# zhoubin-me/agent0

Measured on AMD Instinct MI355X. Metric: env-frames/sec (learner FPS: transitions collected and saved to replay per second with the learner running, pre-frameskip), higher is better.
Workload: dtype f32

## Files before the change

### agent0_amd/csrc/a0_internal.h

```cpp
#pragma once
#include "../../include/agent0_hip.h"
#include "a0_defs.h"

#include <exception>
#if defined(__HIPCC__)
#include <hip/hip_ext.h>
#endif
#include <stdexcept>
#include <string>

int a0_fail(int code, const char* msg);
int a0_fail_hip(int hip_error, const char* what);

struct a0_hip_error : std::runtime_error {
    int err;
    a0_hip_error(int e, const std::string& w) : std::runtime_error(w), err(e) {}
};

#define A0_STR2(x) #x
#define A0_STR(x) A0_STR2(x)
#define A0_HIP_THROW(expr)                                                                                  \
    do {                                                                                                    \
        hipError_t a0_e_ = (expr);                                                                          \
        if (a0_e_ != hipSuccess) throw a0_hip_error((int)a0_e_, std::string(__FILE__ ":" A0_STR(__LINE__) ": ") + hipGetErrorString(a0_e_)); \
    } while (0)

#define A0_TRY try {
#define A0_CATCH                                                   \
    }                                                              \
    catch (const a0_hip_error& e) { return a0_fail_hip(e.err, e.what()); } \
    catch (const std::exception& e) { return a0_fail(A0_EINVAL, e.what()); } \
    catch (...) { return a0_fail(A0_EINVAL, "unknown C++ exception"); }

void a0_trace_push_internal(const char* name);
void a0_trace_pop_internal();
struct a0_trace_scope {
    explicit a0_trace_scope(const char* name) { a0_trace_push_internal(name); }
    ~a0_trace_scope() { a0_trace_pop_internal(); }
    a0_trace_scope(const a0_trace_scope&) = delete;
    a0_trace_scope& operator=(const a0_trace_scope&) = delete;
};

#if defined(__HIPCC__)
bool a0_probe_start(int tag, hipStream_t st);
struct a0_tail_prep;
int a0_conv1_wgrad_fused_launch(const a0_frames_arg* f, int C, int H, int W, int B, const float* d1, float* slabs, const a0_tail_prep* prep, hipStream_t st);
void a0_probe_stop(hipStream_t st, double flops);
bool a0_probe_events(int tag, hipEvent_t* start, hipEvent_t* stop);
void a0_probe_commit(double flops);
int a0_x9_products_now();
#define A0_LAUNCH_PROBED(tag, flops, kern, grid, block, lds, st, ...)                                                              \
    do {                                                                                                                           \
        hipEvent_t a0_e0_ = nullptr, a0_e1_ = nullptr;                                                                             \
        if (a0_probe_events((tag), &a0_e0_, &a0_e1_)) {                                                                            \
            hipExtLaunchKernelGGL(kern, grid, block, (uint32_t)(lds), st, a0_e0_, a0_e1_, 0, __VA_ARGS__);                         \
            a0_probe_commit(flops);                                                                                                \
        } else                                                                                                                     \
            hipLaunchKernelGGL(kern, grid, block, lds, st, __VA_ARGS__);                                                           \
    } while (0)
struct a0_net_core;
int a0_conv23_wgrad_fused_launch(const a0_net_core& n, int B, const float* act1, const float* act2, const float* d2, const float* d3, float* slab2, float* slab3,
                                 hipStream_t st);
#endif
#define A0_TAG_ENCODER_FUSED 12
#define A0_TAG_ENCODER_DGRAD_FUSED 13
#define A0_TAG_ACTOR_STEP_ENC 14
```

### agent0_amd/csrc/conv23_wgrad.hip

```cpp
#include "a0_internal.h"
#include "net_impl.h"

#include <cstdlib>

typedef __bf16 a0q_bf16x8 __attribute__((ext_vector_type(8)));
typedef short a0q_s16x4 __attribute__((ext_vector_type(4)));
typedef uint32_t a0q_u32x2 __attribute__((ext_vector_type(2)));
typedef uint32_t a0q_u32x4 __attribute__((ext_vector_type(4)));
typedef float a0_acc16 __attribute__((ext_vector_type(16)));

constexpr int A0Q_THREADS = 512;
constexpr int A0Q_ROW = 64;

struct a0_c23w_args {
    const float *act1, *act2, *d2, *d3;
    float *slab2, *slab3;
    int B, G2, G3;
};

template <int LAYER> struct a0q_geom;
template <> struct a0q_geom<2> {
    static constexpr int NPOS = 81, STEPS = 5, DROWS = 96, APIX = 100, CIN = 32, K = 512;
    static constexpr int ACT_PLANE = APIX * A0Q_ROW, D_PLANE = 2 * DROWS * A0Q_ROW;
    static constexpr int ACT_F4 = 100 * 8, D_F4 = 81 * 16;
    A0_D static int base_row(int p) { return 10 * (p / 9) + (p % 9); }
};
template <> struct a0q_geom<3> {
    static constexpr int NPOS = 49, STEPS = 3, DROWS = 64, APIX = 81, CIN = 64, K = 576;
    static constexpr int ACT_PLANE = 2 * APIX * A0Q_ROW, D_PLANE = 2 * DROWS * A0Q_ROW;
    static constexpr int ACT_F4 = 81 * 16, D_F4 = 49 * 16;
    A0_D static int base_row(int p) { return 9 * (p / 7) + (p % 7); }
};
constexpr int A0Q_LDS_BYTES = 3 * (a0q_geom<2>::ACT_PLANE + a0q_geom<2>::D_PLANE);
static_assert(3 * (a0q_geom<3>::ACT_PLANE + a0q_geom<3>::D_PLANE) <= A0Q_LDS_BYTES && 2 * A0Q_LDS_BYTES <= 160 * 1024, "conv3 image fits; two workgroups per CU");

A0_D void a0q_split4(const a0_f4& v, a0q_u32x2& hi, a0q_u32x2& mid, a0q_u32x2& lo) {
    const float x[4] = {v.x, v.y, v.z, v.w};
    uint32_t h[4], m[4], l[4];
#pragma unroll
    for (int e = 0; e < 4; ++e) {
        h[e] = __float_as_uint(x[e]);
        const float r1 = x[e] - __uint_as_float(h[e] & 0xffff0000u);
        m[e] = __float_as_uint(r1);
        l[e] = __float_as_uint(r1 - __uint_as_float(m[e] & 0xffff0000u));
    }
    hi.x = __builtin_amdgcn_perm(h[1], h[0], 0x07060302u);  hi.y = __builtin_amdgcn_perm(h[3], h[2], 0x07060302u);
    mid.x = __builtin_amdgcn_perm(m[1], m[0], 0x07060302u); mid.y = __builtin_amdgcn_perm(m[3], m[2], 0x07060302u);
    lo.x = __builtin_amdgcn_perm(l[1], l[0], 0x07060302u);  lo.y = __builtin_amdgcn_perm(l[3], l[2], 0x07060302u);
}

A0_D a0q_u32x4 a0q_frag(const unsigned char* plane, int off0, int off1) {
    typedef __attribute__((address_space(3))) a0q_s16x4 lds_s16x4;
    const a0q_s16x4 k03 = __builtin_amdgcn_ds_read_tr16_b64_v4i16((lds_s16x4*)(plane + off0));
    const a0q_s16x4 k47 = __builtin_amdgcn_ds_read_tr16_b64_v4i16((lds_s16x4*)(plane + off1));
    const a0q_u32x2 a = __builtin_bit_cast(a0q_u32x2, k03), b = __builtin_bit_cast(a0q_u32x2, k47);
    return a0q_u32x4{a.x, a.y, b.x, b.y};
}

template <int NPR, int LAYER, int NT>
A0_D void a0q_mma_steps(const unsigned char* act, const unsigned char* dpl, int aoff, const int (&boff)[a0q_geom<LAYER>::STEPS][2],
                        int a_blk, const int (&b_blk)[2], a0_acc16 (&acc)[2]) {
    typedef a0q_geom<LAYER> G;
    const int lane = threadIdx.x & 63;
    constexpr int TA[9] = {2, 2, 1, 2, 1, 0, 1, 0, 0};
    constexpr int TB[9] = {2, 1, 2, 0, 1, 2, 0, 1, 0};
#pragma unroll
    for (int s = 0; s < G::STEPS; ++s) {
        a0q_u32x4 a[3], b[NT][3];
#pragma unroll
        for (int t = 0; t < 3; ++t) {
            a[t] = a0q_frag(dpl + t * G::D_PLANE + a_blk + s * 16 * A0Q_ROW, aoff, aoff + 4 * A0Q_ROW);
#pragma unroll
            for (int j = 0; j < NT; ++j) b[j][t] = a0q_frag(act + t * G::ACT_PLANE + b_blk[j], boff[s][0], boff[s][1]);
        }
#pragma unroll
        for (int q = 9 - NPR; q < 9; ++q)
#pragma unroll
            for (int j = 0; j < NT; ++j)
                acc[j] = __builtin_amdgcn_mfma_f32_32x32x16_bf16(__builtin_bit_cast(a0q_bf16x8, a[TA[q]]), __builtin_bit_cast(a0q_bf16x8, b[j][TB[q]]), acc[j], 0, 0, 0);
    }
    {
        const int lrow = lane & 31;
        const bool k0 = lane < 32;
        auto f32_at = [](const unsigned char* p, int plane_bytes) {
            const float hi = __uint_as_float((uint32_t)(*(const uint16_t*)p) << 16), mid = __uint_as_float((uint32_t)(*(const uint16_t*)(p + plane_bytes)) << 16),
                        lo = __uint_as_float((uint32_t)(*(const uint16_t*)(p + 2 * plane_bytes)) << 16);
            return (hi + mid) + lo;
        };
        const float av = f32_at(dpl + a_blk + (G::NPOS - 1) * A0Q_ROW + 2 * lrow, G::D_PLANE);
#pragma unroll
        for (int j = 0; j < NT; ++j) {
            const float bv = f32_at(act + b_blk[j] + G::base_row(G::NPOS - 1) * A0Q_ROW + 2 * lrow, G::ACT_PLANE);
            acc[j] = __builtin_amdgcn_mfma_f32_32x32x2f32(k0 ? av : 0.f, k0 ? bv : 0.f, acc[j], 0, 0, 0);
        }
    }
}

template <int NPR, int LAYER>
A0_D void a0q_body(const a0_c23w_args& P, int part, int g, int ngroups, unsigned char* smem) {
    typedef a0q_geom<LAYER> G;
    const int tid = threadIdx.x, lane = tid & 63;
    const int wave = __builtin_amdgcn_readfirstlane(tid >> 6);
    unsigned char* const act = smem;
    unsigned char* const dpl = smem + 3 * G::ACT_PLANE;
    for (int i = tid; i < 3 * G::D_PLANE / 16; i += A0Q_THREADS) ((uint4*)dpl)[i] = uint4{0u, 0u, 0u, 0u};

    int nt, a_blk, b_blk[2], kcol[2], corow;
    if constexpr (LAYER == 2) {
        const int c = wave & 1, th = wave >> 2, tw = (wave >> 1) & 1, kh = (part >> 1) + 2 * th, kw = (part & 1) + 2 * tw;
        nt = 1; a_blk = c * G::DROWS * A0Q_ROW; corow = c * 32;
        b_blk[0] = b_blk[1] = (th * 10 + tw) * A0Q_ROW;
        kcol[0] = kcol[1] = (kh * 4 + kw) * 32;
    } else {
        const int simd = wave & 3, first = 3 * simd + (wave >> 2) * 2;
        nt = wave < 4 ? 2 : 1;
        const int c = first / 6;
        a_blk = c * G::DROWS * A0Q_ROW; corow = c * 32;
#pragma unroll
        for (int j = 0; j < 2; ++j) {
            const int kb = (first + (j < nt ? j : 0)) % 6, kw = kb >> 1, half = kb & 1;
            b_blk[j] = (half * G::APIX + part * 9 + kw) * A0Q_ROW;
            kcol[j] = (part * 3 + kw) * 64 + half * 32;
        }
    }
    const int colb = 2 * (16 * ((lane >> 4) & 1) + 4 * (lane & 3));
    const int aoff = (8 * (lane >> 5) + ((lane & 15) >> 2)) * A0Q_ROW + colb;
    int boff[G::STEPS][2];
#pragma unroll
    for (int s = 0; s < G::STEPS; ++s)
#pragma unroll
        for (int h = 0; h < 2; ++h) {
            const int p = 16 * s + 8 * (lane >> 5) + ((lane & 15) >> 2) + 4 * h;
            boff[s][h] = G::base_row(p) * A0Q_ROW + colb;
        }

    a0_acc16 acc[2];
#pragma unroll
    for (int j = 0; j < 2; ++j)
#pragma unroll
        for (int r = 0; r < 16; ++r) acc[j][r] = 0.f;
    float bsum[4] = {0.f, 0.f, 0.f, 0.f};

    constexpr int RA = (G::ACT_F4 + A0Q_THREADS - 1) / A0Q_THREADS, RD = (G::D_F4 + A0Q_THREADS - 1) / A0Q_THREADS;
    a0_f4 ra[RA], rd[RD];
    auto load_raw = [&](int b) {
        const float* sa = LAYER == 2 ? P.act1 + (long long)b * (400 * 32) : P.act2 + (long long)b * (81 * 64);
#pragma unroll
        for (int j = 0; j < RA; ++j) {
            int i = tid + j * A0Q_THREADS;
            i = i < G::ACT_F4 ? i : G::ACT_F4 - 1;
            if constexpr (LAYER == 2) {
                const int px = i >> 3, r = px / 10, c = px - r * 10;
                ra[j] = *(const a0_f4*)(sa + ((2 * r + (part >> 1)) * 20 + 2 * c + (part & 1)) * 32 + (i & 7) * 4);
            } else ra[j] = *(const a0_f4*)(sa + i * 4);
        }
        const a0_f4* sd = (const a0_f4*)((LAYER == 2 ? P.d2 : P.d3) + (long long)b * (G::NPOS * 64));
#pragma unroll
        for (int j = 0; j < RD; ++j) { const int i = tid + j * A0Q_THREADS; rd[j] = sd[i < G::D_F4 ? i : G::D_F4 - 1]; }
    };
    int b = g;
    if (b < P.B) load_raw(b);
    __syncthreads();
    for (; b < P.B; b += ngroups) {
#pragma unroll
        for (int j = 0; j < RA; ++j) {
            const int i = tid + j * A0Q_THREADS;
            if (i < G::ACT_F4) {
                int row, cb;
                if constexpr (LAYER == 2) { row = i >> 3; cb = (i & 7) * 8; }
                else { const int px = i >> 4, c4 = (i & 15) * 4; row = (c4 >> 5) * G::APIX + px; cb = (c4 & 31) * 2; }
                a0q_u32x2 hi, mid, lo;
                a0q_split4(ra[j], hi, mid, lo);
                unsigned char* d = act + row * A0Q_ROW + cb;
                *(a0q_u32x2*)d = hi; *(a0q_u32x2*)(d + G::ACT_PLANE) = mid; *(a0q_u32x2*)(d + 2 * G::ACT_PLANE) = lo;
            }
        }
#pragma unroll
        for (int j = 0; j < RD; ++j) {
            const int i = tid + j * A0Q_THREADS;
            if (i < G::D_F4) {
                const int c4 = (i & 15) * 4, row = (c4 >> 5) * G::DROWS + (i >> 4), cb = (c4 & 31) * 2;
                bsum[0] += rd[j].x; bsum[1] += rd[j].y; bsum[2] += rd[j].z; bsum[3] += rd[j].w;
                a0q_u32x2 hi, mid, lo;
                a0q_split4(rd[j], hi, mid, lo);
                unsigned char* d = dpl + row * A0Q_ROW + cb;
                *(a0q_u32x2*)d = hi; *(a0q_u32x2*)(d + G::D_PLANE) = mid; *(a0q_u32x2*)(d + 2 * G::D_PLANE) = lo;
            }
        }
        __syncthreads();
        if (b + ngroups < P.B) load_raw(b + ngroups);
        if (nt == 2) a0q_mma_steps<NPR, LAYER, 2>(act, dpl, aoff, boff, a_blk, b_blk, acc);
        else a0q_mma_steps<NPR, LAYER, 1>(act, dpl, aoff, boff, a_blk, b_blk, acc);
        __syncthreads();
    }

    float* out = (LAYER == 2 ? P.slab2 : P.slab3) + (long long)g * (64 * G::K + 64);
#pragma unroll
    for (int j = 0; j < 2; ++j) {
        if (j < nt) {
#pragma unroll
            for (int r = 0; r < 16; ++r) {
                const int row = (r & 3) + 8 * (r >> 2) + 4 * (lane >> 5);
                out[(corow + row) * G::K + kcol[j] + (lane & 31)] = acc[j][r];
            }
        }
    }
    const bool has_bias = part == 0;
    if (has_bias) {
        float* red = (float*)smem;
#pragma unroll
        for (int e = 0; e < 4; ++e) red[tid * 4 + e] = bsum[e];
        __syncthreads();
        constexpr int CH = 64, TPR = CH / 4;
        if (tid < CH) {
            float s = 0.f;
            for (int t = tid >> 2; t < A0Q_THREADS; t += TPR) s += red[t * 4 + (tid & 3)];
            out[64 * G::K + tid] = s;
        }
    }
}

template <int NPR>
__global__ __launch_bounds__(A0Q_THREADS, 4) void a0_conv23_wgrad_fused_kernel(a0_c23w_args P) {
    extern __shared__ __attribute__((aligned(16))) unsigned char a0q_smem[];
    const int xcd = blockIdx.x & 7, k = blockIdx.x >> 3, g = xcd + 8 * (k / 7), part = k % 7;
    if (g >= P.G2) return;
    if (part < 4) a0q_body<NPR, 2>(P, part, g, P.G2, a0q_smem);
    else a0q_body<NPR, 3>(P, part - 4, g, P.G3, a0q_smem);
}

int a0_conv23_wgrad_fused_launch(const a0_net_core& n, int B, const float* act1, const float* act2, const float* d2, const float* d3, float* slab2, float* slab3,
                                 hipStream_t st) {
    int G2 = 0, G3 = 0;
    if (!a0_c23w_plan(n, B, &G2, &G3) || !slab2 || !slab3) return 0;
    a0_c23w_args P;
    P.act1 = act1; P.act2 = act2; P.d2 = d2; P.d3 = d3; P.slab2 = slab2; P.slab3 = slab3; P.B = B; P.G2 = G2; P.G3 = G3;
    const int six = a0_x9_products_now() == 6;
    auto kern = six ? a0_conv23_wgrad_fused_kernel<6> : a0_conv23_wgrad_fused_kernel<9>;
    static bool configured[2] = {false, false};
    if (!configured[six]) {
        A0_HIP_THROW(hipFuncSetAttribute((const void*)kern, hipFuncAttributeMaxDynamicSharedMemorySize, A0Q_LDS_BYTES));
        configured[six] = true;
    }
    if (G2 != G3) return 0;
    hipLaunchKernelGGL(kern, dim3(8 * 7 * ((G2 + 7) / 8)), dim3(A0Q_THREADS), A0Q_LDS_BYTES, st, P);
    A0_HIP_THROW(hipGetLastError());
    return 1;
}
```

### agent0_amd/csrc/encoder_fused.hip

```cpp
#include "a0_internal.h"
#include "net_tables.h"
#include "operands.h"
#include "update_tail.h"

#include <cstdlib>
#include <type_traits>

typedef float a0_acc4 __attribute__((ext_vector_type(4)));

struct a0_fused_args {
    const uint8_t* frames; const int* slot; long long sample_stride; int chan_off;
    const float *wt1, *wt2, *wt3;
    const float *wx2, *wx3;
    const float *b1, *b2, *b3;
    float *act1, *act2, *act3;
    int B;
    int C, H, W, H1, W1, H2, W2, H3, W3;
    int off_act1, off_act2, off_end;
    int rp1, rp2;
};

A0_HD void a0_fused_set_wt(a0_fused_args& P, const float* wt, int C) {
    const a0_wt_layout T{C};
    P.wt1 = wt + T.conv1x(); P.wt2 = wt + T.conv2(); P.wt3 = wt + T.conv3(); P.wx2 = wt + T.conv2x(); P.wx3 = wt + T.conv3x();
// ... 879 lines not shown
    static size_t configured[2] = {0, 0};
    if (lds > configured[six]) {
        if (hipFuncSetAttribute((const void*)kern, hipFuncAttributeMaxDynamicSharedMemorySize, (int)lds) != hipSuccess)
            return a0_fail(A0_EINVAL, "a0_actor_qhead_env_step_enc: LDS");
        configured[six] = lds;
    }
    A0_LAUNCH_PROBED(A0_TAG_ACTOR_STEP_ENC, 2.0 * (400.0 * 32 * 256 + 81.0 * 64 * 512 + 49.0 * 64 * 576) * Q.E, kern, dim3(Q.E), dim3(A0_FUSED_THREADS), lds, st, Q, N);
    return a0_fail_hip((int)hipGetLastError(), "a0_actor_qhead_env_step_enc");
}

struct a0_fused_multi_args { a0_fused_args p[3]; int first[4]; };
template <int ORD>
__global__ __launch_bounds__(A0_FUSED_THREADS) void a0_encoder_fused_multi_kernel(a0_fused_multi_args M) {
    const int bid = (int)blockIdx.x;
    const int k = bid >= M.first[2] ? 2 : (bid >= M.first[1] ? 1 : 0);
    a0_encoder_fused_x9_body<ORD, true>(M.p[k], bid - M.first[k], M.first[k + 1] - M.first[k]);
}

template <int MBW1, int MBW2, int MBW3, int WC, bool X9, bool LOOP, int ORD>
__global__ __launch_bounds__(A0_FUSED_THREADS) void a0_encoder_fused_kernel(a0_fused_args P) {
    if constexpr (X9) {
        static_assert(MBW1 == 7 && MBW2 == 3 && MBW3 == 2 && WC == 84, "the split-operand body is written for the 4 x 84 x 84 geometry");
        a0_encoder_fused_x9_body<ORD, LOOP>(P, (int)blockIdx.x, (int)gridDim.x);
        return;
    }
    extern __shared__ __attribute__((aligned(16))) unsigned char smem[];
    uint16_t* img = (uint16_t*)smem;
    float* fl = (float*)smem;
    float* act1 = fl + P.off_act1;
    float* act2 = fl + P.off_act2;
    const int obs_bytes = P.C * P.H * P.W;
    const int M1 = P.H1 * P.W1, M2 = P.H2 * P.W2, M3 = P.H3 * P.W3;
    a0_wring1<A0_R1> ring1;
    a0_wring<64, 4, A0_R2> ring2;
    a0_wring<64, 4, A0_R3> ring3;
    ring1.init(P.wt1, P.C);
    ring2.init(P.wt2, 512);
    ring3.init(P.wt3, 576);
    ring1.prologue();
    constexpr int OW1 = WC == 84 ? 20 : 0, OW2 = WC == 84 ? 9 : 0;
    a0_pre<32, 2, MBW1, EpiFwd<OW1>> pre1;
    a0_pre<64, 4, MBW2, EpiFwd<OW2>> pre2;
    a0_pre<64, 4, MBW3, EpiFwd<0>> pre3;
    pre1.load(EpiFwd<OW1>{P.b1, nullptr, 0, 0, 1, nullptr, 32}, M1);
    pre2.load(EpiFwd<OW2>{P.b2, nullptr, 0, 0, 1, nullptr, 64}, M2);
    pre3.load(EpiFwd<0>{P.b3, nullptr, 0, 0, 1, nullptr, 64}, M3);
    for (int b = blockIdx.x; b < P.B; b += gridDim.x) {
        const long long s = P.slot ? (long long)P.slot[b] : (long long)b;
        const uint4* src = (const uint4*)(P.frames + s * P.sample_stride + P.chan_off);
        constexpr int TRIPS = 4;
        const int n16 = obs_bytes >> 4;
        for (int i0 = threadIdx.x; i0 < n16; i0 += TRIPS * A0_FUSED_THREADS) {
            uint4 v[TRIPS];
#pragma unroll
            for (int j = 0; j < TRIPS; ++j) {
                const int i = i0 + j * A0_FUSED_THREADS;
                v[j] = src[i < n16 ? i : n16 - 1];
            }
#pragma unroll
            for (int j = 0; j < TRIPS; ++j) {
                const int i = i0 + j * A0_FUSED_THREADS;
                a0_bytes16_to_img(img, i < n16 ? i : n16 - 1, v[j]);
            }
        }
        __syncthreads();
        const EpiFwd<OW1> e1{P.b1, act1, A0_P1, P.rp1, P.W1, P.act1 ? P.act1 + (long long)b * M1 * 32 : nullptr, 32};
        const int wmg1 = __builtin_amdgcn_readfirstlane(threadIdx.x >> 6) / 2;
        if (MBW1 > 1 && wmg1 + (MBW1 - 1) * 4 >= ((M1 + 15) >> 4))
            a0_conv1_stage<(MBW1 > 1 ? MBW1 - 1 : 1), A0_R1, WC>(img, P.H * P.W, P.W, P.W1, M1, ring1, e1, pre1, [&] { ring2.prologue(); });
        else
            a0_conv1_stage<MBW1, A0_R1, WC>(img, P.H * P.W, P.W, P.W1, M1, ring1, e1, pre1, [&] { ring2.prologue(); });
        AF2 f2{act1, P.rp1, P.W2};
        const EpiFwd<OW2> e2{P.b2, act2, A0_P2, P.rp2, P.W2, P.act2 ? P.act2 + (long long)b * M2 * 64 : nullptr, 64};
        a0_conv_stage<64, 4, MBW2, 3, A0_R2>(f2, M2, 512, ring2, e2, pre2, [&] { ring3.prologue(); });
        AF3 f3{act2, P.rp2, P.W3};
        const EpiFwd<0> e3{P.b3, nullptr, 0, 0, 1, P.act3 + (long long)b * M3 * 64, 64};
        a0_conv_stage<64, 4, MBW3, 3, A0_R3>(f3, M3, 576, ring3, e3, pre3, [&] { ring1.prologue(); });
    }
}

struct a0_dgrad_args {
    const float *d3, *act1, *act2;
    float *d2, *d1;
    const float *wd3, *wd2;
    int B;
};
constexpr int A0_RPDA = 11 * A0_P2X + 96, A0_RPDB = 11 * A0_P2X + 48;
constexpr int A0_DTERMA = 11 * A0_RPDA, A0_DTERMB = 11 * A0_RPDB;
struct AFD3X {
    static constexpr int term = A0_DTERMA;
    const uint16_t* planes;
    A0_D int row(int m) const { const int oh = m / 9, ow = m - oh * 9; return oh * A0_RPDA + ow * A0_P2X; }
    A0_D int step_off(int st) const { const int tap = st >> 1; return (tap / 3) * A0_RPDA + (tap % 3) * A0_P2X + 32 * (st & 1); }
};
struct AFD2X {
    static constexpr int term = A0_DTERMB;
    const uint16_t* planes;
    A0_D int row(int m) const { const int oh = m / 10, ow = m - oh * 10; return oh * A0_RPDB + ow * A0_P2X; }
    A0_D int step_off(int st) const { const int cell = st >> 1; return (cell >> 1) * A0_RPDB + (cell & 1) * A0_P2X + 32 * (st & 1); }
};
struct EpiBwd3X {
    static constexpr bool PER_ELEM = true;
    static constexpr bool ROW4 = false;
    static constexpr bool TR = true;
    const float* mask; float* dst; uint16_t* planes;
    A0_D a0_f4 pre_elem4(int m, int n0) const { return *(const a0_f4*)(mask + (unsigned)(m * 64 + n0)); }
    A0_D void emit_n4(int m, int n0, const a0_acc4& acc, const float* pre) const {
        float v[4];
#pragma unroll
        for (int r = 0; r < 4; ++r) v[r] = pre[r] > 0.f ? acc[r] : 0.f;
        *(a0_f4*)(dst + (unsigned)(m * 64 + n0)) = a0_f4{v[0], v[1], v[2], v[3]};
        uint2 hi, mid, lo;
        a0_split4(v, hi, mid, lo);
        const int oh = m / 9, ow = m - oh * 9;
        uint16_t* d = planes + (oh + 1) * A0_RPDB + (ow + 1) * A0_P2X + n0;
        *(uint2*)d = hi; *(uint2*)(d + A0_DTERMB) = mid; *(uint2*)(d + 2 * A0_DTERMB) = lo;
    }
};
static_assert((A0_RPDB % 4) == 0 && (A0_DTERMB % 4) == 0 && (A0_P2X % 4) == 0, "8-byte aligned plane writes");
struct EpiBwdPair {
    static constexpr bool PER_ELEM = true;
    static constexpr bool ROW4 = false;
    static constexpr bool TR = true;
    const float* mask; float* dst; int p0;
    A0_D unsigned gi(int m, int n0) const {
        const int p = p0 + (n0 >> 5), oh = m / 10, ow = m - oh * 10;
        return (unsigned)(((oh * 2 + (p >> 1)) * 20 + ow * 2 + (p & 1)) * 32 + (n0 & 31));
    }
    A0_D a0_f4 pre_elem4(int m, int n0) const { return *(const a0_f4*)(mask + gi(m, n0)); }
    A0_D void emit_n4(int m, int n0, const a0_acc4& acc, const float* pre) const {
        *(a0_f4*)(dst + gi(m, n0)) = a0_f4{pre[0] > 0.f ? acc[0] : 0.f, pre[1] > 0.f ? acc[1] : 0.f, pre[2] > 0.f ? acc[2] : 0.f, pre[3] > 0.f ? acc[3] : 0.f};
    }
};
template <int ORD>
__global__ __launch_bounds__(A0_FUSED_THREADS) void a0_encoder_dgrad_fused_x9_kernel(a0_dgrad_args P) {
    extern __shared__ __attribute__((aligned(16))) unsigned char smem[];
    uint16_t* plA = (uint16_t*)smem;
    uint16_t* plB = plA + 3 * A0_DTERMA;
    for (int i = threadIdx.x; i < 3 * (A0_DTERMA + A0_DTERMB) / 2; i += A0_FUSED_THREADS) ((uint32_t*)smem)[i] = 0u;
    float* const xch0 = (float*)(smem + 3 * (A0_DTERMA + A0_DTERMB) * 2);
    float* const xch1 = xch0 + 4 * 4 * 256;
    const int lane = threadIdx.x & 63, wave = __builtin_amdgcn_readfirstlane(threadIdx.x >> 6), wn = wave & 3, wk = wave >> 2;
    a0_wring9<64, 4, 3, 2> ring3;
    a0_wring9<64, 4, 2, 2> ringq[2];
    ring3.init(P.wd3, 576);
    ring3.prologue();
    const uint4* const wq = (const uint4*)P.wd2 + (((wn & 1) * 16 + (lane & 15)) * 4 + (lane >> 4)) * 3 + (wn >> 1) * 3072 + wk * 384;
    __syncthreads();
    for (int b = blockIdx.x; b < P.B; b += gridDim.x) {
        const a0_f4* src = (const a0_f4*)(P.d3 + (long long)b * 49 * 64);
        for (int i = threadIdx.x; i < 49 * 16; i += A0_FUSED_THREADS) {
            const a0_f4 v = src[i];
            const int pos = i >> 4, c4 = (i & 15) * 4, h = pos / 7, w = pos - h * 7;
            const float x[4] = {v.x, v.y, v.z, v.w};
            uint2 hi, mid, lo;
            a0_split4(x, hi, mid, lo);
            uint16_t* d = plA + (h + 2) * A0_RPDA + (w + 2) * A0_P2X + c4;
            *(uint2*)(d) = hi; *(uint2*)(d + A0_DTERMA) = mid; *(uint2*)(d + 2 * A0_DTERMA) = lo;
        }
        __syncthreads();
        const AFD3X f3{plA};
        const AFD2X f2{plB};
        const EpiBwd3X e3{P.act2 + (long long)b * 81 * 64, P.d2 + (long long)b * 81 * 64, plB};
        const EpiBwdPair e2a{P.act1 + (long long)b * 400 * 32, P.d1 + (long long)b * 400 * 32, 0};
        const EpiBwdPair e2b{P.act1 + (long long)b * 400 * 32, P.d1 + (long long)b * 400 * 32, 2};
        a0_conv_stage_x9k<ORD, 64, 4, 6, 3, 1>(f3, 81, ring3, e3, xch0, xch1, [&] { ringq[0].init_at(wq, 4, 768); ringq[0].prologue(); });
        a0_conv_stage_x9k<ORD, 64, 4, 7, 2, 4>(f2, 100, ringq[0], e2a, xch0, xch1, [&] { ringq[1].init_at(wq + 2 * 3072, 4, 768); ringq[1].prologue(); });
        a0_conv_stage_x9k<ORD, 64, 4, 7, 2, 4>(f2, 100, ringq[1], e2b, xch0, xch1, [&] { ring3.prologue(); });
    }
}

__global__ void a0_conv_wt_kernel(const float* __restrict__ w1, const float* __restrict__ w2, const float* __restrict__ w3, float* __restrict__ wt, int K1,
                                  float* __restrict__ wt2, const int* __restrict__ state, int* __restrict__ commit) {
    const bool mirror = wt2 != nullptr && state[4] != 0;
    if (commit != nullptr && blockIdx.x == 0 && threadIdx.x == 0) { commit[1] = commit[5]; commit[0] = 0; }
    const a0_wt_layout T{K1 / 64};
    const int i = blockIdx.x * blockDim.x + threadIdx.x;
    if (i >= T.total()) return;
    uint32_t out = 0;
    if (i >= T.conv2() && i < T.conv2x()) {
        const bool c3 = i >= T.conv3();
        const int e = i - (c3 ? T.conv3() : T.conv2());
        const int j = e & 3, q = (e >> 2) & 3, n = (e >> 4) & 63, k = 16 * (e >> 10) + 4 * j + q;
        out = __float_as_uint(c3 ? w3[n * 576 + k] : w2[n * 512 + k]);
    } else {
        enum { CONV1, CONV2, CONV3, DGRAD3, DGRAD2 } seg;
        int e, N = 64, phase = 0;
        if (i < T.conv2()) { seg = CONV1; e = i; N = 32; }
        else if (i < T.conv3x()) { seg = CONV2; e = i - T.conv2x(); }
        else if (i < T.dgrad3x()) { seg = CONV3; e = i - T.conv3x(); }
        else if (i < T.dgrad2x()) { seg = DGRAD3; e = i - T.dgrad3x(); }
        else { seg = DGRAD2; e = i - T.dgrad2x(); phase = e / T.n_dgrad2x_phase; e -= phase * T.n_dgrad2x_phase; N = 32; }
        const int pair = e & 3, f = e >> 2, s = f % 3, q = (f / 3) & 3, n = (f / 12) % N, t = f / (12 * N);
        for (int h = 0; h < 2; ++h) {
            const int k = 32 * t + 8 * q + 2 * pair + h, cell = k >> 6, co = k & 63;
            float w;
            if (seg == CONV1) w = w1[n * K1 + k] / 255.0f;
            else if (seg == CONV2) w = w2[n * 512 + k];
            else if (seg == CONV3) w = w3[n * 576 + k];
            else if (seg == DGRAD3) {
                const int kh = 2 - cell / 3, kw = 2 - cell % 3;
                w = w3[co * 576 + (kh * 3 + kw) * 64 + n];
            } else {
                const int kh = (phase >> 1) + 2 * (1 - (cell >> 1)), kw = (phase & 1) + 2 * (1 - (cell & 1));
                w = w2[co * 512 + (kh * 4 + kw) * 32 + n];
            }
            out |= a0_bf16_term(w, s) << (16 * h);
        }
    }
    *(uint32_t*)(wt + i) = out;
    if (mirror) *(uint32_t*)(wt2 + i) = out;
}

extern "C" long long a0_net_conv_wt_floats(int C) { return a0_wt_layout{C}.total(); }

extern "C" int a0_net_conv_wt_refresh(const a0_encoder_weights* w, int C, float* wt, void* stream) {
    if (!w || !w->w1 || !w->w2 || !w->w3 || !wt || C < 1) return a0_fail(A0_EINVAL, "a0_net_conv_wt_refresh: bad argument");
    const long long n = a0_net_conv_wt_floats(C);
    hipLaunchKernelGGL(a0_conv_wt_kernel, dim3((unsigned)((n + 255) / 256)), dim3(256), 0, (hipStream_t)stream, w->w1, w->w2, w->w3, wt, C * 64, (float*)nullptr,
                       (const int*)nullptr, (int*)nullptr);
    return a0_fail_hip((int)hipGetLastError(), "a0_net_conv_wt_refresh");
}

extern "C" int a0_net_conv_wt_refresh_sync(const a0_encoder_weights* w, int C, float* wt, float* wt_target, const int* state, void* stream) {
    if (!w || !w->w1 || !w->w2 || !w->w3 || !wt || !wt_target || !state || C < 1) return a0_fail(A0_EINVAL, "a0_net_conv_wt_refresh_sync: bad argument");
    const long long n = a0_net_conv_wt_floats(C);
    hipLaunchKernelGGL(a0_conv_wt_kernel, dim3((unsigned)((n + 255) / 256)), dim3(256), 0, (hipStream_t)stream, w->w1, w->w2, w->w3, wt, C * 64, wt_target, state, (int*)nullptr);
    return a0_fail_hip((int)hipGetLastError(), "a0_net_conv_wt_refresh_sync");
}

int a0_conv_wt_refresh_commit(const a0_encoder_weights* w, int C, float* wt, float* wt_target, int* state, hipStream_t st) {
    if (!w || !w->w1 || !w->w2 || !w->w3) return a0_fail(A0_EINVAL, "a0_adam_step_sync_wt: encoder weights missing");
    const long long n = a0_net_conv_wt_floats(C);
    hipLaunchKernelGGL(a0_conv_wt_kernel, dim3((unsigned)((n + 255) / 256)), dim3(256), 0, st, w->w1, w->w2, w->w3, wt, C * 64, wt_target, (const int*)state, state);
    return a0_fail_hip((int)hipGetLastError(), "a0_adam_step_sync_wt");
}

static bool a0_fused_layout(int C, int H, int W, a0_fused_args& P, size_t& lds_bytes) {
    a0_net_core n;
    if (!a0_net_core_init(n, C, H, W)) return false;
    const int M1 = n.H1 * n.W1, M2 = n.H2 * n.W2, M3 = n.H3 * n.W3;
    if (M1 > 7 * 4 * 16 || M2 > 4 * 2 * 16 || M3 > 2 * 2 * 16) return false;
    if ((C * 2) % A0_R1 || (W & 3)) return false;
    const int obs_bytes = C * H * W;
    if (obs_bytes % 16) return false;
    P.C = C; P.H = H; P.W = W; P.H1 = n.H1; P.W1 = n.W1; P.H2 = n.H2; P.W2 = n.W2; P.H3 = n.H3; P.W3 = n.W3;
// ... 22 lines not shown
    a0_fused_args P; size_t lds;
    return a0_fused_layout(C, H, W, P, lds) ? 1 : 0;
}

extern "C" int a0_net_encoder_fwd_fused(int C, int H, int W, const float* wt, const a0_encoder_weights* w, const a0_frames_arg* f, int B,
                                        float* act1, float* act2, float* act3, void* stream) {
    A0_TRY
    if (!wt || !w || !w->b1 || !w->b2 || !w->b3 || !f || !f->frames || !act3 || B < 1) return a0_fail(A0_EINVAL, "a0_net_encoder_fwd_fused: bad argument");
    a0_fused_args P;
    size_t lds = 0;
    if (!a0_fused_fill(C, H, W, wt, w, f, act1, act2, act3, B, P, lds)) return a0_fail(A0_EINVAL, "a0_net_encoder_fwd_fused: observation shape not supported by the fused kernel");
    if ((f->sample_stride % 16) || (f->chan_off % 16) || (((uintptr_t)f->frames) % 16)) return a0_fail(A0_EINVAL, "a0_net_encoder_fwd_fused: frames must be 16-byte aligned");
    const int mb1 = (P.H1 * P.W1 + 15) / 16, mb2 = (P.H2 * P.W2 + 15) / 16, mb3 = (P.H3 * P.W3 + 15) / 16;
    const bool standard = ((mb1 + 3) / 4 == 7) && ((mb2 + 1) / 2 == 3) && ((mb3 + 1) / 2 == 2) && W == 84;
    const bool x9 = standard && H == 84 && C == 4;
    int which = x9 ? 2 : (standard ? 1 : 0);
    if (x9) lds = A0_X9_LDS_BYTES;
    static_assert(3 * 9 * A0_RP2X * 2 <= 2 * 4 * 84 * 84, "the act2 term planes fit into the dead image");
    const int gridx = (which == 2 && B > 256) ? 256 : B;
    if (which == 2 && gridx < B) which = 3;
    static size_t configured[6] = {0, 0, 0, 0, 0, 0};
    const int six = a0_x9_products_now() == 6;
    if (six && which >= 2) which += 2;
    typedef void (*a0_enc_kern)(a0_fused_args);
    const a0_enc_kern fn = which == 5 ? a0_encoder_fused_kernel<7, 3, 2, 84, true, true, 2> : which == 4 ? a0_encoder_fused_kernel<7, 3, 2, 84, true, false, 2>
                         : which == 3 ? a0_encoder_fused_kernel<7, 3, 2, 84, true, true> : which == 2 ? a0_encoder_fused_kernel<7, 3, 2, 84, true>
                         : which == 1 ? a0_encoder_fused_kernel<7, 3, 2, 84, false> : a0_encoder_fused_kernel<7, 4, 2, 0, false>;
    if (lds > configured[which]) {
        A0_HIP_THROW(hipFuncSetAttribute((const void*)fn, hipFuncAttributeMaxDynamicSharedMemorySize, (int)lds));
        configured[which] = lds;
    }
    const double per_obs = 2.0 * ((double)P.H1 * P.W1 * 32 * (P.C * 64) + (double)P.H2 * P.W2 * 64 * 512 + (double)P.H3 * P.W3 * 64 * 576);
    A0_LAUNCH_PROBED(A0_TAG_ENCODER_FUSED, per_obs * B, fn, dim3((which == 3 || which == 5) ? gridx : B), dim3(A0_FUSED_THREADS), lds, (hipStream_t)stream, P);
    A0_HIP_THROW(hipGetLastError());
    return A0_OK;
    A0_CATCH
}

extern "C" int a0_net_encoder_fwd_fused_multi(int C, int H, int W, int n, const a0_encoder_pass* pass, void* stream) {
    A0_TRY
    if (n < 1 || n > 3 || !pass) return a0_fail(A0_EINVAL, "a0_net_encoder_fwd_fused_multi: 1 to 3 passes");
    if (!(C == 4 && H == 84 && W == 84)) return a0_fail(A0_EINVAL, "a0_net_encoder_fwd_fused_multi: 4 x 84 x 84 observations on the split-operand kernel only");
    a0_fused_multi_args M;
    size_t lds = 0;
    long long total = 0;
    for (int i = 0; i < n; ++i) {
        const a0_encoder_pass& q = pass[i];
        if (!q.wt || !q.w || !q.w->b1 || !q.w->b2 || !q.w->b3 || !q.f || !q.f->frames || !q.act3 || q.B < 1) return a0_fail(A0_EINVAL, "a0_net_encoder_fwd_fused_multi: bad pass");
        if ((q.f->sample_stride % 16) || (q.f->chan_off % 16) || (((uintptr_t)q.f->frames) % 16)) return a0_fail(A0_EINVAL, "a0_net_encoder_fwd_fused_multi: frames must be 16-byte aligned");
        if (!a0_fused_fill(C, H, W, q.wt, q.w, q.f, q.act1, q.act2, q.act3, q.B, M.p[i], lds))
            return a0_fail(A0_EINVAL, "a0_net_encoder_fwd_fused_multi: observation shape");
        total += q.B;
    }
    for (int i = n; i < 3; ++i) M.p[i] = M.p[0];
    int grid = (int)(total < 256 ? total : 256), used = 0;
    if (grid < n) grid = n;
    for (int i = 0; i < n; ++i) {
        M.first[i] = used;
        int share = (i == n - 1) ? grid - used : (int)((long long)grid * pass[i].B / total);
        if (share < 1) share = 1;
        if (share > pass[i].B) share = pass[i].B;
        used += share;
    }
    for (int i = n; i <= 3; ++i) M.first[i] = 0x7fffffff;
    M.first[n] = used;
    lds = A0_X9_LDS_BYTES;
    const int six = a0_x9_products_now() == 6;
    auto kern = six ? a0_encoder_fused_multi_kernel<2> : a0_encoder_fused_multi_kernel<4>;
    static bool configured[2] = {false, false};
    if (!configured[six]) {
        A0_HIP_THROW(hipFuncSetAttribute((const void*)kern, hipFuncAttributeMaxDynamicSharedMemorySize, (int)lds));
        configured[six] = true;
    }
    const a0_fused_args& P0 = M.p[0];
    const double per_obs = 2.0 * ((double)P0.H1 * P0.W1 * 32 * (P0.C * 64) + (double)P0.H2 * P0.W2 * 64 * 512 + (double)P0.H3 * P0.W3 * 64 * 576);
    A0_LAUNCH_PROBED(A0_TAG_ENCODER_FUSED, per_obs * (double)total, kern, dim3(used), dim3(A0_FUSED_THREADS), lds, (hipStream_t)stream, M);
    A0_HIP_THROW(hipGetLastError());
    return A0_OK;
    A0_CATCH
}

extern "C" int a0_net_encoder_dgrad_fused_supported(int C, int H, int W) { return (C >= 1 && H == 84 && W == 84) ? 1 : 0; }

extern "C" int a0_net_encoder_dgrad_fused(int C, int H, int W, const float* wt, const float* d3, const float* act1, const float* act2, int B, float* d2,
                                          float* d1, void* stream) {
    A0_TRY
    if (!wt || !d3 || !act1 || !act2 || !d2 || !d1 || B < 1) return a0_fail(A0_EINVAL, "a0_net_encoder_dgrad_fused: bad argument");
    if (!a0_net_encoder_dgrad_fused_supported(C, H, W)) return a0_fail(A0_EINVAL, "a0_net_encoder_dgrad_fused: 84x84 observations only");
    a0_dgrad_args P;
    P.d3 = d3; P.act1 = act1; P.act2 = act2; P.d2 = d2; P.d1 = d1; P.B = B;
    P.wd3 = wt + a0_wt_layout{C}.dgrad3x(); P.wd2 = wt + a0_wt_layout{C}.dgrad2x();
    const size_t lds = (size_t)3 * (A0_DTERMA + A0_DTERMB) * 2 + (4 * 4 + 4 * 3) * 1024;
    static bool configured[2] = {false, false};
    const int six = a0_x9_products_now() == 6;
    auto fn = six ? a0_encoder_dgrad_fused_x9_kernel<2> : a0_encoder_dgrad_fused_x9_kernel<4>;
    if (!configured[six]) {
        A0_HIP_THROW(hipFuncSetAttribute((const void*)fn, hipFuncAttributeMaxDynamicSharedMemorySize, (int)lds));
        configured[six] = true;
    }
    const int gridx = B > 256 ? 256 : B;
    A0_LAUNCH_PROBED(A0_TAG_ENCODER_DGRAD_FUSED, 2.0 * (81.0 * 64 * 576 + 400.0 * 32 * 256) * B, fn, dim3(gridx), dim3(A0_FUSED_THREADS), lds, (hipStream_t)stream, P);
    A0_HIP_THROW(hipGetLastError());
    return A0_OK;
    A0_CATCH
}
```

### agent0_amd/csrc/learner.hip

```cpp
#include "learner_state.h"

extern "C" int a0_learner_create(const a0_learner_desc* d, a0_learner** out) { return a0_learner_create_on(d, nullptr, out); }

extern "C" int a0_learner_set_rng(a0_learner* L, int stream_id, unsigned long long offset) {
    if (!L || stream_id < 0 || stream_id > 7 || (offset & 3)) return a0_fail(A0_EINVAL, "a0_learner_set_rng: stream 0..7, offset a multiple of four");
    L->rng.off[stream_id] = offset;
    return A0_OK;
}

extern "C" int a0_learner_rng_state(a0_learner* L, unsigned long long* words, int set) {
    if (!L || !words) return a0_fail(A0_EINVAL, "a0_learner_rng_state: null argument");
    if (set) {
        for (int i = 0; i < 8; ++i) if (words[1 + i] & 3) return a0_fail(A0_EINVAL, "a0_learner_rng_state: offsets are multiples of four");
        L->rng.seed = words[0];
        for (int i = 0; i < 8; ++i) L->rng.off[i] = words[1 + i];
    } else {
        words[0] = L->rng.seed;
        for (int i = 0; i < 8; ++i) words[1 + i] = L->rng.off[i];
    }
    return A0_OK;
}

extern "C" int a0_learner_create_on(const a0_learner_desc* d, const a0_learner_buffers* bufs, a0_learner** out) {
    A0_TRY
// ... 5 lines not shown
        (d->algo != A0_ALGO_DQN && d->algo != A0_ALGO_C51 && d->algo != A0_ALGO_IQN && d->algo != A0_ALGO_FQF && d->algo != A0_ALGO_QR && d->algo != A0_ALGO_MDQN))
        return a0_fail(A0_EINVAL, "a0_learner_create: bad description");
    if (d->algo == A0_ALGO_QR && (d->num_atoms < 1 || d->num_atoms > 1024)) return a0_fail(A0_EINVAL, "a0_learner_create: qr needs 1 <= num_atoms <= 1024");
    if (d->algo == A0_ALGO_MDQN && !(d->mdqn_tau > 0.0)) return a0_fail(A0_EINVAL, "a0_learner_create: mdqn needs tau > 0");
    if (d->algo == A0_ALGO_FQF && (d->fqf_F < 2 || d->fqf_F > 32 || d->A + (d->dueling ? 1 : 0) > 32))
        return a0_fail(A0_EINVAL, "a0_learner_create: fqf needs 2 <= F <= 32, A + dueling <= 32");
    if (d->algo == A0_ALGO_IQN && (d->iqn_K < 1 || d->iqn_N < 1 || d->iqn_N_dash < 1 || d->A + (d->dueling ? 1 : 0) > 32))
        return a0_fail(A0_EINVAL, "a0_learner_create: iqn needs K, N, N' >= 1, A + dueling <= 32");
    if (d->algo == A0_ALGO_DQN && d->A + (d->dueling ? 1 : 0) > 24)
        return a0_fail(A0_EINVAL, "a0_learner_create: the dqn handle covers scalar heads with A + dueling <= 24 actions");
    if (d->algo == A0_ALGO_C51 && (d->num_atoms < 2 || d->num_atoms > 64 || !(d->vmax > d->vmin)))
        return a0_fail(A0_EINVAL, "a0_learner_create: c51 needs 2 <= num_atoms <= 64 and vmin < vmax");
    a0_learner* L = new a0_learner();
    try {
        L->d = *d;
        a0_net_desc nd{4, 84, 84};
        if (a0_net_create(&nd, &L->net) != A0_OK) { delete L; return A0_EINVAL; }
        const bool c51 = d->algo == A0_ALGO_C51;
        L->T = (c51 || d->algo == A0_ALGO_QR) ? d->num_atoms : 1;
        L->Nq = d->A * L->T;
        L->V = d->dueling ? L->T : 0;
        L->NQ = d->A + (d->dueling ? 1 : 0);
        L->Npad = (int)ceil_to(L->Nq + L->V, 32);
        {
            const int Ron = d->double_q ? 2 * d->B : d->B;
            L->qr_fused = d->algo == A0_ALGO_QR && d->A <= 32 && (3LL * L->Npad + ceil_to(L->T, 4)) * 4 <= 150 * 1024 &&
                          std::max(a0_dense_fwd_partial_slabs(Ron, L->Npad, 512), a0_dense_fwd_partial_slabs(d->B, L->Npad, 512)) <= 8;
            L->mdqn_fused = d->algo == A0_ALGO_MDQN && L->NQ <= 24;
        }
        const bool dist = c51 || L->qr_fused;
        const bool generic = (d->algo == A0_ALGO_QR && !L->qr_fused) || (d->algo == A0_ALGO_MDQN && !L->mdqn_fused);
        long long off = 0;
        auto add = [&](Blk& b, int N, int K) { b = Blk{off, N, K}; off += b.size(); };
        add(L->conv1, 32, L->C * 64); add(L->conv2, 64, 512); add(L->conv3, 64, 576);
        if (d->noisy) { add(L->fc1, 512, L->feat); add(L->fc1_sigma, 512, L->feat); add(L->head, L->Npad, 512); add(L->head_sigma, L->Npad, 512); }
        else { add(L->fc1, 512, L->feat); add(L->head, L->Npad, 512); }
        const bool fqf = d->algo == A0_ALGO_FQF;
        const bool iqn = d->algo == A0_ALGO_IQN || fqf;
        if (iqn) add(L->cos, L->feat, 64);
        L->n_adam = off;
        if (fqf) { add(L->frac, 32, L->feat); L->F = d->fqf_F; }
        if (d->noisy) {
            L->eff_fc1 = Blk{0, 512, L->feat};
            L->eff_head = Blk{L->eff_fc1.size(), L->Npad, 512};
            L->n_eff = L->eff_fc1.size() + L->eff_head.size();
            long long no = 0;
            auto mod = [&](int block, int r0, int r1, int in_f) {
                a0_noise_mod m{block, r0, r1, in_f, 0, 0, 0};
                m.off_in = no; no += ceil_to(in_f, 4);
                m.off_w = no; no += ceil_to(r1 - r0, 4);
                m.off_b = no; no += ceil_to(r1 - r0, 4);
                L->mods[L->n_mods++] = m;
            };
            mod(0, 0, 512, L->feat);
            mod(1, 0, L->Nq, 512);
            if (d->dueling) mod(1, L->Nq, L->Nq + L->V, 512);
            L->noise_len = no;
            L->rng.init(d->seed, 0);
        }
        L->n_pad = ceil_to(off, 4);
        L->wt_floats = a0_net_conv_wt_floats(L->C);
        L->gamma_n = (float)std::pow(d->discount, (double)d->n_step);
        const int B = d->B;
        L->online = U.online ? U.online : L->alloc<float>(L->n_pad, true); L->target = U.target ? U.target : L->alloc<float>(L->n_pad, true);
        L->grads = U.grads ? U.grads : L->alloc<float>(L->n_pad + 4, true);
        L->m = U.adam_m ? U.adam_m : L->alloc<float>(L->n_pad, true); L->v = U.adam_v ? U.adam_v : L->alloc<float>(L->n_pad, true);
        L->state = U.state ? U.state : L->alloc<int>(8, true); L->scalars = U.scalars ? U.scalars : L->alloc<float>(4, true);
        L->loss_ring = U.loss_ring ? U.loss_ring : L->alloc<float>(1024, true); L->loss_ring_cap = U.loss_ring ? U.loss_ring_cap : 1024;
        L->wt_on = U.wt_online ? U.wt_online : L->alloc<float>(L->wt_floats, true); L->wt_tg = U.wt_target ? U.wt_target : L->alloc<float>(L->wt_floats, true);
        L->act1 = L->alloc<float>((long long)B * L->H1 * L->W1 * 32); L->act2 = L->alloc<float>((long long)B * L->H2 * L->W2 * 64);
        L->act3_t = L->alloc<float>((long long)B * L->feat);
        L->ns_fc1 = a0_dense_fwd_partial_slabs(B, 512, L->feat);
        if (!dist) {
            L->act3_o = L->alloc<float>((long long)B * L->feat);
            if (d->double_q || L->mdqn_fused) L->act3_s = L->alloc<float>((long long)B * L->feat);
            for (int i = 0; i < ((d->double_q || L->mdqn_fused) ? 3 : 2); ++i) L->fc1_slabs[i] = L->alloc<float>((long long)L->ns_fc1 * B * 512);
            L->h = L->alloc<float>((long long)B * 512);
            if (L->mdqn_fused) L->q_cur = L->alloc<float>((long long)B * d->A);
        }
        L->q_o = L->alloc<float>((long long)B * d->A * L->T); L->q_t = L->alloc<float>((long long)B * d->A * L->T);
        const long long Rg = fqf ? (long long)B * d->fqf_F : (iqn ? (long long)B * d->iqn_N : (long long)B);
        L->draw = L->alloc<float>(Rg * L->Npad); L->dh = L->alloc<float>(Rg * 512); L->d3 = L->alloc<float>((long long)B * L->feat);
        L->d2 = L->alloc<float>((long long)B * L->H2 * L->W2 * 64); L->d1 = L->alloc<float>((long long)B * L->H1 * L->W1 * 32); L->loss = L->alloc<float>(B);
        const long long s_head = ceil_to(a0_dense_wgrad_scratch((int)Rg, L->Npad, 512), 4), s_fc1 = ceil_to(a0_dense_wgrad_scratch((int)Rg, 512, L->feat), 4);
        const long long s_cos = iqn ? ceil_to(a0_dense_wgrad_scratch((int)Rg, L->feat, 64), 4) : 0;
        L->slab_off[0] = 0; L->slab_off[1] = s_head;
        L->slab_off3[0] = 0; L->slab_off3[1] = s_head; L->slab_off3[2] = s_head + s_fc1;
        L->enc_slab_off = s_head + s_fc1 + s_cos;
        long long n_slab = L->enc_slab_off + a0_net_encoder_bwd_scratch(L->net, B);
        if (fqf && a0_dense_wgrad_scratch(B, 32, L->feat) > n_slab) n_slab = a0_dense_wgrad_scratch(B, 32, L->feat);
        L->slabs = L->alloc<float>(n_slab > 4 ? n_slab : 4);
        if (d->noisy) {
            L->eff_on = U.eff_online ? U.eff_online : L->alloc<float>(L->n_eff, true); L->eff_tg = U.eff_target ? U.eff_target : L->alloc<float>(L->n_eff, true);
            if (U.noise) L->noise = U.noise;
            else {
            L->noise = L->alloc<float>(2 * L->noise_len, true);
            const unsigned long long o = L->rng.reserve(4, L->noise_len);
            (void)L->rng.reserve(4, L->noise_len);
            if (a0_rng_normal(L->rng.seed, 4, o, 0.1f, L->noise, 2 * L->noise_len, nullptr) != A0_OK) { delete L; return A0_EINVAL; }
            A0_HIP_THROW(hipDeviceSynchronize());
            }
        }
        if (dist) {
            const int dq = d->double_q ? 1 : 0;
            L->R_on = dq ? 2 * B : B;
            L->ns_on = a0_dense_fwd_partial_slabs(L->R_on, 512, L->feat);
            L->nh_on = a0_dense_fwd_partial_slabs(L->R_on, L->Npad, 512);
            L->nh_tg = a0_dense_fwd_partial_slabs(B, L->Npad, 512);
            L->act3_on = L->alloc<float>((long long)L->R_on * L->feat);
            L->act3_o = L->act3_on;
            if (dq) L->act3_s = L->act3_on + (long long)B * L->feat;
            L->fc1_on = L->alloc<float>((long long)L->ns_on * L->R_on * 512); L->fc1_tg = L->alloc<float>((long long)L->ns_fc1 * B * 512);
            L->h_on = L->alloc<float>((long long)L->R_on * 512); L->h_tg = L->alloc<float>((long long)B * 512);
            L->h = L->h_on;
            L->hs_on = L->alloc<float>((long long)L->nh_on * L->R_on * L->Npad); L->hs_tg = L->alloc<float>((long long)L->nh_tg * B * L->Npad);
            L->a_star = L->alloc<int>(B, true);
        }
        if (L->qr_fused) {
            L->qr_taus = L->alloc<float>(L->T);
            std::vector<float> t((size_t)L->T);
            for (int i = 0; i < L->T; ++i) t[(size_t)i] = (2.0f * (float)i + 1.0f) / (2.0f * (float)L->T);
            A0_HIP_THROW(hipMemcpy(L->qr_taus, t.data(), (size_t)L->T * 4, hipMemcpyHostToDevice));
        }
        if (c51) {
            L->atoms = L->alloc<float>(L->T); L->m_proj = L->alloc<float>((long long)B * L->T);
            std::vector<float> at((size_t)L->T);
            const float lo = (float)d->vmin, hi = (float)d->vmax, step = (hi - lo) / (float)(L->T - 1);
            for (int i = 0; i < L->T; ++i) at[(size_t)i] = i < L->T / 2 ? std::fmaf(step, (float)i, lo) : std::fmaf(-step, (float)(L->T - 1 - i), hi);
            A0_HIP_THROW(hipMemcpy(L->atoms, at.data(), (size_t)L->T * 4, hipMemcpyHostToDevice));
        }
        if (generic) {
            const long long nq = (long long)B * d->A * L->T;
            auto gw = [&](a0_learner::DWs& w, float* act3, float* h, float* q) { w.act3 = act3; w.h = h ? h : L->alloc<float>((long long)B * 512); w.raw = L->alloc<float>((long long)B * L->Npad); w.q = q ? q : L->alloc<float>(nq); };
            gw(L->go, L->act3_o, L->h, L->q_o);
            gw(L->gt, L->act3_t, nullptr, L->q_t);
            if (d->double_q && d->algo == A0_ALGO_QR) gw(L->gs, L->act3_s ? L->act3_s : (L->act3_s = L->alloc<float>((long long)B * L->feat)), nullptr, nullptr);
            if (d->algo == A0_ALGO_MDQN) gw(L->gm, L->alloc<float>((long long)B * L->feat), nullptr, nullptr);
            L->g_dq = L->alloc<float>(nq, true);
            L->a_star = L->alloc<int>(B, true);
            const long long s1 = a0_dense_fwd_scratch(B, 512, L->feat), s2 = a0_dense_fwd_scratch(B, L->Npad, 512);
            L->fwd_scratch = L->alloc<float>(std::max(4LL, std::max(s1, s2)));
            if (d->algo == A0_ALGO_QR) {
                L->y = L->alloc<float>((long long)B * L->T);
                L->qr_taus = L->alloc<float>(L->T);
                std::vector<float> t((size_t)L->T);
                for (int i = 0; i < L->T; ++i) t[(size_t)i] = (2.0f * (float)i + 1.0f) / (2.0f * (float)L->T);
                A0_HIP_THROW(hipMemcpy(L->qr_taus, t.data(), (size_t)L->T * 4, hipMemcpyHostToDevice));
            }
        }
        if (iqn) {
            const int K = fqf ? d->fqf_F : d->iqn_K, N = fqf ? d->fqf_F : d->iqn_N, Nd = fqf ? d->fqf_F : d->iqn_N_dash;
            L->rng.init(d->seed, 0);
            L->a_star = L->alloc<int>(B, true);
            long long sc = 4;
            auto ws = [&](a0_learner::QWs& w, int n_tau, float* act3, bool grads) {
                w.n_tau = n_tau; w.R = (long long)B * n_tau; w.act3 = act3;
                w.h = L->alloc<float>(w.R * 512); w.raw = L->alloc<float>(w.R * L->Npad); w.q = L->alloc<float>(w.R * d->A);
                w.cosx = L->alloc<float>(w.R * 64); w.emb = L->alloc<float>(w.R * L->feat); w.x = L->alloc<float>(w.R * L->feat);
                if (grads) { w.dq = L->alloc<float>(w.R * d->A, true); w.dx = L->alloc<float>(w.R * L->feat); w.demb = L->alloc<float>(w.R * L->feat); }
                for (int r : {B * K, B * Nd, B * N, B * (N - 1)}) {
                    if (r > w.R || r < 1) continue;
                    const long long a = a0_dense_fwd_scratch(r, L->feat, 64), b2 = a0_dense_fwd_scratch(r, 512, L->feat), c = a0_dense_fwd_scratch(r, L->Npad, 512);
                    sc = std::max(sc, std::max(a, std::max(b2, c)));
                }
            };
            ws(L->qo, N, L->act3_o, true);
// ... 349 lines not shown
        const float* Ws[3] = {L->Wf(false), L->Wf(true), W3};
        A0_CHECK(a0_dense_fwd_partial_multi(n_fc1, Xs, L->feat, Ws, B, 512, L->feat, L->fc1_slabs, nullptr, stream));
        ns = a0_dense_fwd_partial_multi_slabs(n_fc1, B, 512, L->feat);
    } else {
        A0_CHECK(a0_dense_fwd_partial(L->act3_t, L->feat, L->Wf(true), B, 512, L->feat, L->fc1_slabs[1], stream));
        if (third) A0_CHECK(a0_dense_fwd_partial(L->act3_s, L->feat, W3, B, 512, L->feat, L->fc1_slabs[2], stream));
        A0_CHECK(a0_dense_fwd_partial(L->act3_o, L->feat, L->Wf(false), B, 512, L->feat, L->fc1_slabs[0], stream));
    }
    if (mdqn)
        A0_CHECK(a0_mdqn_head_loss_slabs(L->fc1_slabs[0], L->fc1_slabs[1], L->fc1_slabs[2], (long long)B * 512, ns, L->bf(false), L->bf(true), L->h, L->Wh(false), L->bh(false),
                                         L->Wh(true), L->bh(true), A, L->d.dueling ? 1 : 0, L->Npad, act, rew, done, wgt, L->gamma_n, (float)L->d.mdqn_tau, (float)L->d.mdqn_lo, B,
                                         L->loss, L->q_o, L->q_t, L->q_cur, L->draw, L->state, L->dh, stream));
    else
    A0_CHECK(a0_dqn_head_loss_slabs(L->fc1_slabs[0], L->fc1_slabs[1], dq ? L->fc1_slabs[2] : nullptr, (long long)B * 512, ns, L->bf(false), L->bf(true), L->h,
                                    L->Wh(false), L->bh(false), L->Wh(true), L->bh(true), A, L->d.dueling ? 1 : 0, L->Npad, act, rew, done, wgt, L->gamma_n, B,
                                    L->loss, L->q_o, L->q_t, L->draw, L->state, L->dh, stream));
    }
    const bool quantile = L->d.algo == A0_ALGO_IQN || L->d.algo == A0_ALGO_FQF;
    if (quantile) {
        const int N = L->qo.n_tau;
        const int R = (int)L->qo.R;
        A0_CHECK(a0_dueling_bwd(L->qo.dq, L->draw, L->Npad, R, A, 1, L->d.dueling ? 1 : 0, stream));
        A0_CHECK(a0_dense_dgrad(L->draw, L->Wh(false), L->qo.h, L->dh, R, L->Npad, 512, stream));
        if (a0_dense_dgrad_hadamard_ok(R, 512, L->feat, N)) {
            A0_CHECK(a0_dense_dgrad_hadamard(L->dh, L->Wf(false), L->qo.emb, L->act3_o, L->qo.demb, L->d3, R, 512, L->feat, N, stream));
        } else {
            A0_CHECK(a0_dense_dgrad(L->dh, L->Wf(false), nullptr, L->qo.dx, R, 512, L->feat, stream));
            A0_CHECK(a0_hadamard_bwd(L->qo.dx, L->qo.emb, L->act3_o, L->qo.demb, L->d3, B, N, L->feat, stream));
        }
        {
            const float* dY[3] = {L->draw, L->dh, L->qo.demb};
            const float* X[3] = {L->qo.h, L->qo.x, L->qo.cosx};
            const int ldx[3] = {512, L->feat, 64}, Rr[3] = {R, R, R}, Nn[3] = {L->Npad, 512, L->feat}, Kk[3] = {512, L->feat, 64};
            float* G[3] = {L->grads + L->head.off, L->grads + L->fc1.off, L->grads + L->cos.off};
            A0_CHECK(a0_dense_wgrad_multi(3, dY, X, ldx, G, Rr, Nn, Kk, L->slabs, L->slab_off3, pp, stream));
        }
    }
    if (!quantile) {
        const float* dY[2] = {L->draw, L->dh};
        const float* X[2] = {L->h, L->act3_o};
        const int ldx[2] = {512, L->feat}, R[2] = {B, B}, N[2] = {L->Npad, 512}, K[2] = {512, L->feat};
        float* G[2] = {L->grads + L->head.off, L->grads + L->fc1.off};
        if (head_wgrad_done) {
            if (a0_dense_dgrad_wgrad_ok(B, 512, L->feat)) {
                A0_CHECK(a0_dense_dgrad_wgrad(L->dh, L->Wf(false), L->act3_o, L->feat, L->d3, G[1], B, 512, L->feat, stream));
            } else {
                A0_CHECK(a0_dense_dgrad(L->dh, L->Wf(false), L->act3_o, L->d3, B, 512, L->feat, stream));
                A0_CHECK(a0_dense_wgrad_multi(1, dY + 1, X + 1, ldx + 1, G + 1, R + 1, N + 1, K + 1, L->slabs, L->slab_off + 1, pp, stream));
            }
        } else if (a0_dense_dgrad_wgrad2_ok(B, 512, L->feat, L->Npad, 512)) {
            A0_CHECK(a0_dense_dgrad_wgrad2(L->dh, L->Wf(false), L->act3_o, L->feat, L->d3, G[1], B, 512, L->feat, L->draw, L->h, 512, G[0], L->Npad, 512, stream));
        } else if (a0_dense_dgrad_wgrad_ok(B, 512, L->feat)) {
            A0_CHECK(a0_dense_dgrad_wgrad(L->dh, L->Wf(false), L->act3_o, L->feat, L->d3, G[1], B, 512, L->feat, stream));
            A0_CHECK(a0_dense_wgrad_multi(1, dY, X, ldx, G, R, N, K, L->slabs, L->slab_off, pp, stream));
        } else {
            A0_CHECK(a0_dense_dgrad(L->dh, L->Wf(false), L->act3_o, L->d3, B, 512, L->feat, stream));
            A0_CHECK(a0_dense_wgrad_multi(2, dY, X, ldx, G, R, N, K, L->slabs, L->slab_off, pp, stream));
        }
    }
    auto sigma_grads = [&]() -> int {
        const float *gmu[3], *nin[3], *nw[3], *nb[3];
        float* gs[3];
        int N[3], K[3], r0[3], r1[3];
        for (int k = 0; k < L->n_mods; ++k) {
            const a0_noise_mod& m = L->mods[k];
            const Blk &bm = m.block ? L->head : L->fc1, &bs = m.block ? L->head_sigma : L->fc1_sigma;
            gmu[k] = L->grads + bm.off; gs[k] = L->grads + bs.off; N[k] = bm.N; K[k] = bm.K; r0[k] = m.r0; r1[k] = m.r1;
            nin[k] = L->noise + m.off_in; nw[k] = L->noise + m.off_w; nb[k] = L->noise + m.off_b;
        }
        return a0_noisy_multi(1, L->n_mods, gmu, nullptr, gs, N, K, r0, r1, nin, nw, nb, stream);
    };
    const long long conv_end = L->fc1.off;
    if (dp) {
        if (L->d.noisy) A0_CHECK(sigma_grads());
        A0_CHECK(a0_nan_flag_export(L->state, L->grads + L->n_pad, stream));
        if (dp_inline) {
            A0_CHECK(a0_dp_allreduce(L->dp_comm, L->grads + conv_end, L->n_pad + 1 - conv_end, stream));
        } else {
            A0_HIP_THROW(hipEventRecord(L->dp_ev[0], (hipStream_t)stream));
            A0_HIP_THROW(hipStreamWaitEvent(L->dp_side, L->dp_ev[0], 0));
            A0_CHECK(a0_dp_allreduce(L->dp_comm, L->grads + conv_end, L->n_pad + 1 - conv_end, L->dp_side));
        }
    }
    A0_CHECK(a0_net_encoder_dgrad_fused(L->C, L->H, L->W, L->wt_on, L->d3, L->act1, L->act2, B, L->d2, L->d1, stream));
    a0_update_tail_plan tail;
    const bool fuse_tail = !dp && L->clip_max_norm <= 0.f && !(L->d.noisy && pend.n > 0);
    if (fuse_tail)
        A0_CHECK(a0_net_encoder_wgrad_tail(L->net, &w_on, &f_obs, B, L->act1, L->act2, L->d3, L->d2, L->d1, L->grads + L->conv1.off, L->grads + L->conv2.off,
                                           L->grads + L->conv3.off, L->slabs + L->enc_slab_off, &pend, &tail, L->state, L->scalars, L->d.lr, 0.9, 0.999,
                                           hard_freq, stream));
    else
    A0_CHECK(a0_net_encoder_wgrad(L->net, &w_on, &f_obs, B, L->act1, L->act2, L->d3, L->d2, L->d1, L->grads + L->conv1.off, L->grads + L->conv2.off, L->grads + L->conv3.off,
                                  L->slabs + L->enc_slab_off, &pend, stream));
    if (dp) {
        if (dp_inline) {
            A0_CHECK(a0_dp_allreduce(L->dp_comm, L->grads, conv_end, stream));
        } else {
            A0_HIP_THROW(hipEventRecord(L->dp_ev[1], (hipStream_t)stream));
            A0_HIP_THROW(hipStreamWaitEvent(L->dp_side, L->dp_ev[1], 0));
            A0_CHECK(a0_dp_allreduce(L->dp_comm, L->grads, conv_end, L->dp_side));
            A0_HIP_THROW(hipEventRecord(L->dp_ev[2], L->dp_side));
            A0_HIP_THROW(hipStreamWaitEvent((hipStream_t)stream, L->dp_ev[2], 0));
        }
    } else if (L->d.noisy) {
        A0_CHECK(sigma_grads());
    }
    if (loss_out) A0_HIP_THROW(hipMemcpyAsync(loss_out, L->loss, (size_t)B * 4, hipMemcpyDeviceToDevice, (hipStream_t)stream));
    if (L->d.algo == A0_ALGO_FQF)
        A0_CHECK(a0_rmsprop_step(on + L->frac.off, L->grads + L->frac.off, L->rms_sq, L->frac.size(), L->d.lr / 2e4, 0.95, 1e-5, L->d.max_grad_norm > 0.0 ? L->d.max_grad_norm : -1.0, L->clip, stream));
    const double eps = L->d.adam_eps > 0.0 ? L->d.adam_eps : 1e-2 / (double)B;
    if (fuse_tail) {
        A0_CHECK(a0_update_tail(on, L->grads, L->m, L->v, L->n_adam, L->state, L->scalars, 0.9, 0.999, eps, tg, L->n_pad, &tail, &w_on, L->C, L->wt_on, L->wt_tg, L->loss, B,
                                L->loss_ring, L->loss_ring_cap, stream));
        return blend();
    }
    if (L->clip_max_norm > 0.f) {
        A0_CHECK(a0_grad_norm_partials(L->grads, L->n_adam, L->gnorm_partials, stream));
        A0_CHECK(a0_adam_step_sync_wt_clip(on, L->grads, L->m, L->v, L->n_adam, L->state, L->scalars, L->d.lr, 0.9, 0.999, eps, hard_freq, tg, L->n_pad, dp ? L->grads + L->n_pad : nullptr, &w_on, L->C,
                                           L->wt_on, L->wt_tg, L->loss, B, L->loss_ring, L->loss_ring_cap, L->gnorm_partials, L->clip_max_norm, L->gnorm_ring, L->gnorm_ring_cap, stream));
        return blend();
    }
    A0_CHECK(a0_adam_step_sync_wt(on, L->grads, L->m, L->v, L->n_adam, L->state, L->scalars, L->d.lr, 0.9, 0.999, eps, hard_freq, tg, L->n_pad, dp ? L->grads + L->n_pad : nullptr, &w_on, L->C,
                                  L->wt_on, L->wt_tg, L->loss, B, L->loss_ring, L->loss_ring_cap, stream));
    return blend();
    A0_CATCH
}
```

### agent0_amd/csrc/learner_state.h

```cpp
#pragma once
#include "a0_internal.h"

#include <cmath>
#include <vector>

struct Blk { long long off; int N, K; long long w() const { return off; } long long b() const { return off + (long long)N * K; } long long size() const { return (long long)N * K + N; } };

static inline long long ceil_to(long long x, long long m) { return (x + m - 1) / m * m; }

struct a0_host_rng {
    unsigned long long seed = 0;
    unsigned long long off[8] = {0, 0, 0, 0, 0, 0, 0, 0};
    void init(unsigned long long s, unsigned rank) { seed = (s & 0xFFFFFFFFull) | ((unsigned long long)(rank & 0xFFFFu) << 32); }
    unsigned long long reserve(int stream, long long n) { const unsigned long long o = off[stream]; off[stream] += (unsigned long long)((n + 3) / 4 * 4); return o; }
    unsigned next_seed32(int stream) { const unsigned long long o = reserve(stream, 4); return (unsigned)((seed * 0x9E3779B1ull + o * 0x85EBCA77ull + (unsigned long long)stream) & 0xFFFFFFFFull); }
};

struct a0_noise_mod { int block; int r0, r1, in_f; long long off_in, off_w, off_b; };

struct a0_learner {
    a0_learner_desc d;
    a0_net* net = nullptr;
    int C = 4, H = 84, W = 84, H1 = 20, W1 = 20, H2 = 9, W2 = 9, feat = 3136, Npad = 32, NQ = 0;
    Blk conv1, conv2, conv3, fc1, head;
    int T = 1, Nq = 0, V = 0;
    Blk fc1_sigma, head_sigma;
    Blk eff_fc1, eff_head;
    long long n_eff = 0, noise_len = 0;
    int n_mods = 0;
    a0_noise_mod mods[3];
    a0_host_rng rng;
    float *eff_on = nullptr, *eff_tg = nullptr, *noise = nullptr;
    float *atoms = nullptr, *m_proj = nullptr;
    int* a_star = nullptr;
    float *act3_on = nullptr, *fc1_on = nullptr, *fc1_tg = nullptr, *h_on = nullptr, *h_tg = nullptr, *hs_on = nullptr, *hs_tg = nullptr;
    int R_on = 0, ns_on = 1, nh_on = 1, nh_tg = 1;
    Blk cos;
    struct QWs { int n_tau = 0; long long R = 0; float *h = nullptr, *raw = nullptr, *q = nullptr, *cosx = nullptr, *emb = nullptr, *x = nullptr, *act3 = nullptr;
                 float *dq = nullptr, *dx = nullptr, *demb = nullptr; } qo, qt, qs;
    float *t_sel = nullptr, *t_tgt = nullptr, *t_on = nullptr, *y = nullptr, *fwd_scratch = nullptr;
    Blk frac;
    int F = 0;
    struct FWs { float *logits = nullptr, *tau_all = nullptr, *tau_hat = nullptr; } fo, ft, fs;
    QWs qf;
    float *inner_taus = nullptr, *rms_sq = nullptr, *frac_loss = nullptr, *dfrac = nullptr, *clip = nullptr;
    struct DWs { float *act3 = nullptr, *h = nullptr, *raw = nullptr, *q = nullptr; } go, gt, gs, gm;
    float *g_dq = nullptr, *qr_taus = nullptr;
    bool qr_fused = false, mdqn_fused = false;
    float* q_cur = nullptr;
    long long slab_off3[3] = {0, 0, 0};
    const float* Wf(bool tg) const { return d.noisy ? (tg ? eff_tg : eff_on) + eff_fc1.w() : (tg ? target : online) + fc1.w(); }
    const float* bf(bool tg) const { return d.noisy ? (tg ? eff_tg : eff_on) + eff_fc1.b() : (tg ? target : online) + fc1.b(); }
    const float* Wh(bool tg) const { return d.noisy ? (tg ? eff_tg : eff_on) + eff_head.w() : (tg ? target : online) + head.w(); }
    const float* bh(bool tg) const { return d.noisy ? (tg ? eff_tg : eff_on) + eff_head.b() : (tg ? target : online) + head.b(); }
    long long n_adam = 0, n_pad = 0, wt_floats = 0;
    float gamma_n = 0.f;
    int ns_fc1 = 1;
    long long slab_off[2] = {0, 0}, enc_slab_off = 0;
    int loss_ring_cap = 1024;
    float clip_max_norm = 0.f;
    double* gnorm_partials = nullptr;
    float* gnorm_ring = nullptr;
    int gnorm_ring_cap = 0;
    double target_tau = 0.0;
    bool updated = false;
    float *online = nullptr, *target = nullptr, *grads = nullptr, *m = nullptr, *v = nullptr, *scalars = nullptr, *loss_ring = nullptr;
    float *wt_on = nullptr, *wt_tg = nullptr;
    int* state = nullptr;
    float *act1 = nullptr, *act2 = nullptr, *act3_o = nullptr, *act3_t = nullptr, *act3_s = nullptr;
    float *fc1_slabs[3] = {nullptr, nullptr, nullptr};
    float *h = nullptr, *q_o = nullptr, *q_t = nullptr, *draw = nullptr, *dh = nullptr, *d3 = nullptr, *d2 = nullptr, *d1 = nullptr, *loss = nullptr, *slabs = nullptr;
    std::vector<void*> owned;
    long long dp_comm = 0;
    hipStream_t dp_side = nullptr;
    bool dp_one_rank = false;
    hipEvent_t dp_ev[3] = {nullptr, nullptr, nullptr};

    template <class T> T* alloc(long long n, bool zero = false) {
        void* p = nullptr;
        A0_HIP_THROW(hipMalloc(&p, (size_t)(n > 0 ? n : 1) * sizeof(T)));
        owned.push_back(p);
        if (zero) A0_HIP_THROW(hipMemset(p, 0, (size_t)(n > 0 ? n : 1) * sizeof(T)));
        return (T*)p;
    }
    ~a0_learner() {
        for (void* p : owned) (void)hipFree(p);
        if (net) a0_net_destroy(net);
        for (hipEvent_t e : dp_ev) if (e) (void)hipEventDestroy(e);
        if (dp_side) (void)hipStreamDestroy(dp_side);
    }
    a0_encoder_weights enc(const float* flat) const { return a0_encoder_weights{flat + conv1.w(), flat + conv1.b(), flat + conv2.w(), flat + conv2.b(), flat + conv3.w(), flat + conv3.b()}; }
};

#define A0_CHECK(call) do { int a0_rc_ = (call); if (a0_rc_ != A0_OK) return a0_rc_; } while (0)
```

### agent0_amd/csrc/net.hip

```cpp
#include "igemm_x9.h"
#include "short_k_fwd.h"
#include "a0_internal.h"
#include "net_impl.h"
#include "update_tail.h"

#include <vector>

__global__ __launch_bounds__(256) void a0_reduce_slabs_kernel(const float* __restrict__ slabs, long long slab_stride, int nslab,
                                                               float* __restrict__ out, long long count) {
    __shared__ float red[8][33];
    const int c = threadIdx.x & 31, g = threadIdx.x >> 5;
    const long long i = (long long)blockIdx.x * 32 + c;
    float s = 0.f;
    if (i < count)
        for (int z = g; z < nslab; z += 8) s += slabs[(long long)z * slab_stride + i];
    red[g][c] = s;
    __syncthreads();
    if (g == 0 && i < count) {
        float t = 0.f;
#pragma unroll
        for (int j = 0; j < 8; ++j) t += red[j][c];
        out[i] = t;
    }
}
// ... 88 lines not shown

struct a0_probe_t {
    int tag = 0;
    std::vector<hipEvent_t> ev;
    size_t used = 0;
    double flops = 0.0;
};
static a0_probe_t g_probe;

bool a0_probe_start(int tag, hipStream_t st) {
    if (g_probe.tag == 0 || g_probe.tag != tag || g_probe.used + 2 > g_probe.ev.size()) return false;
    return hipEventRecord(g_probe.ev[g_probe.used], st) == hipSuccess;
}
void a0_probe_stop(hipStream_t st, double flops) {
    (void)hipEventRecord(g_probe.ev[g_probe.used + 1], st);
    g_probe.used += 2;
    g_probe.flops += flops;
}

bool a0_probe_events(int tag, hipEvent_t* start, hipEvent_t* stop) {
    if (g_probe.tag == 0 || g_probe.tag != tag || g_probe.used + 2 > g_probe.ev.size()) return false;
    *start = g_probe.ev[g_probe.used]; *stop = g_probe.ev[g_probe.used + 1];
    return true;
}
void a0_probe_commit(double flops) { g_probe.used += 2; g_probe.flops += flops; }

extern "C" int a0_probe_begin(int tag, int max_launches) {
    A0_TRY
    for (hipEvent_t e : g_probe.ev) (void)hipEventDestroy(e);
    g_probe.ev.clear();
    g_probe.used = 0; g_probe.flops = 0.0; g_probe.tag = 0;
    if (tag <= 0 || max_launches <= 0) return A0_OK;
    g_probe.ev.resize(2 * (size_t)max_launches);
    for (auto& e : g_probe.ev) A0_HIP_THROW(hipEventCreate(&e));
    g_probe.tag = tag;
    return A0_OK;
    A0_CATCH
}

extern "C" int a0_probe_end(double* host_out3) {
    A0_TRY
    if (!host_out3) return a0_fail(A0_EINVAL, "a0_probe_end: null");
    double ms = 0.0;
    for (size_t i = 0; i + 1 < g_probe.used; i += 2) {
        A0_HIP_THROW(hipEventSynchronize(g_probe.ev[i + 1]));
        float t = 0.f;
        A0_HIP_THROW(hipEventElapsedTime(&t, g_probe.ev[i], g_probe.ev[i + 1]));
        ms += t;
    }
    host_out3[0] = (double)(g_probe.used / 2); host_out3[1] = ms; host_out3[2] = g_probe.flops;
    g_probe.tag = 0;
    return A0_OK;
    A0_CATCH
}

static int g_gemm_x9 = (getenv("A0_GEMM") && std::string(getenv("A0_GEMM")) == "fp32") ? 0 : 1;
static constexpr long long A0_X9_BIG_TILES = 256;
extern "C" int a0_gemm_mode(int mode) {
    const int prev = g_gemm_x9;
    if (mode >= 0) g_gemm_x9 = mode ? 1 : 0;
    return prev;
}

static int g_x9_products = (getenv("A0_X9_PRODUCTS") && atoi(getenv("A0_X9_PRODUCTS")) == 9) ? 9 : 6;
int a0_x9_products_now() { return g_x9_products; }
extern "C" int a0_x9_products(int n) {
    const int prev = g_x9_products;
    if (n == 6 || n == 9) g_x9_products = n;
    return prev;
}

static constexpr long long A0_X9_HUGE_TILES = 250;
template <class OP> struct a0_is_mat { static constexpr bool value = false; };
template <> struct a0_is_mat<OpMatKC> { static constexpr bool value = true; };
template <> struct a0_is_mat<OpMatXC> { static constexpr bool value = true; };
template <class OP> struct a0_is_gather { static constexpr bool value = false; };
template <> struct a0_is_gather<OpActXC> { static constexpr bool value = true; };

struct a0_hip_backend {
    hipStream_t st;
    int tag = 0;
    const a0_tail_prep* prep = nullptr;
    bool prep_done = false;
    template <class OA, class OB, class EP, int WM, int WN, int MT, int NT>
    void igemm(const typename OA::Params& pa, const typename OB::Params& pb, const typename EP::Params& pe, int X, int Y, int K, int splits) {
        hipEvent_t e0 = nullptr, e1 = nullptr;
        const bool probe = a0_probe_events(tag, &e0, &e1);
        bool carried = false;
        const bool x9 = g_gemm_x9 != 0;
        constexpr bool eight = WM * WN == 8;
        constexpr int FWM = eight ? WM : WM, FWN = eight ? WN / 2 : WN, FMT = MT, FNT = eight ? NT * 2 : NT;
        static_assert(!eight || (WN % 2) == 0, "eight-wave shapes: even wave count along N");
        if constexpr (a0_x9_ok<OA>::value && a0_x9_ok<OB>::value) {
            const int sp = splits < 1 ? 1 : splits;
            const long long big = (long long)((X + 127) / 128) * ((Y + 127) / 128) * sp;
            constexpr bool wgrad_family = OA::MODE == A0_XC;
            const bool deep = K / sp >= 512;
            const bool large = X >= 128 && Y >= 128 && big >= A0_X9_BIG_TILES && (deep || !wgrad_family);
            constexpr bool mats = a0_is_mat<OA>::value && a0_is_mat<OB>::value;
            const long long huge = (long long)((X + 255) / 256) * ((Y + 127) / 128) * sp;
            const double fill_huge = (double)huge / (256.0 * (double)((huge + 255) / 256)), fill_big = (double)big / (256.0 * (double)((big + 255) / 256));
            if constexpr (mats) {
                if (x9 && X >= 256 && Y >= 128 && huge >= A0_X9_HUGE_TILES && fill_huge >= 0.93 * fill_big && (deep || !wgrad_family)) {
                    A0_HIP_THROW((a0_igemm_x9_launch<OA, OB, EP, 4, 2, 2, 2, 1>(st, pa, pb, pe, X, Y, K, splits, e0, e1)));
                    if (probe) a0_probe_commit(2.0 * (double)X * (double)Y * (double)K);
                    return;
                }
            }
            if (x9 && large) { A0_HIP_THROW((a0_igemm_x9_launch<OA, OB, EP, 4, 2, 1, 2>(st, pa, pb, pe, X, Y, K, splits, e0, e1))); carried = true; }
            else if (x9 && (!wgrad_family || (deep && !a0_is_gather<OB>::value))) { A0_HIP_THROW((a0_igemm_x9_launch<OA, OB, EP, WM, WN, MT, NT>(st, pa, pb, pe, X, Y, K, splits, e0, e1))); carried = true; }
            else {
                if (probe) A0_HIP_THROW(hipEventRecord(e0, st));
                A0_HIP_THROW((a0_igemm_launch<OA, OB, EP, FWM, FWN, FMT, FNT>(st, pa, pb, pe, X, Y, K, splits)));
            }
        } else {
            if (probe) A0_HIP_THROW(hipEventRecord(e0, st));
            A0_HIP_THROW((a0_igemm_launch<OA, OB, EP, FWM, FWN, FMT, FNT>(st, pa, pb, pe, X, Y, K, splits)));
        }
        if (probe) {
            if (!carried) A0_HIP_THROW(hipEventRecord(e1, st));
            a0_probe_commit(2.0 * (double)X * (double)Y * (double)K);
        }
    }
    void short_k_fwd(const float* X, int ldx, const float* W, const float* b, const float* M, int group, float* Y, float* Y2, int R, int N, int relu) {
        A0_HIP_THROW(a0_short_k_fwd_launch(st, X, ldx, W, b, M, group, Y, Y2, R, N, relu));
    }
    int conv1_wgrad_fused(const a0_net_core& n, const a0_frames_arg& f, int B, const float* d1, float* slabs) {
        if (!slabs) return 0;
        const bool probe = g_probe.tag != 0 && g_probe.tag == tag && g_probe.used + 2 <= g_probe.ev.size();
        if (probe) A0_HIP_THROW(hipEventRecord(g_probe.ev[g_probe.used], st));
        const int g = a0_conv1_wgrad_fused_launch(&f, n.C, n.H, n.W, B, d1, slabs, prep, st);
        if (g > 0 && prep) prep_done = true;
        if (probe && g > 0) {
            A0_HIP_THROW(hipEventRecord(g_probe.ev[g_probe.used + 1], st));
            g_probe.used += 2;
            g_probe.flops += 2.0 * 32.0 * (double)n.K1 * (double)B * n.H1 * n.W1;
        }
        return g;
    }
    bool conv23_wgrad_fused(const a0_net_core& n, int B, const float* act1, const float* act2, const float* d2, const float* d3, float* slab2, float* slab3) {
        const bool probe = g_probe.tag != 0 && g_probe.tag == A0_TAG_CONV2_WGRAD && g_probe.used + 2 <= g_probe.ev.size();
        if (probe) A0_HIP_THROW(hipEventRecord(g_probe.ev[g_probe.used], st));
        const int ran = a0_conv23_wgrad_fused_launch(n, B, act1, act2, d2, d3, slab2, slab3, st);
        if (probe && ran) {
            A0_HIP_THROW(hipEventRecord(g_probe.ev[g_probe.used + 1], st));
            g_probe.used += 2;
            g_probe.flops += 2.0 * 64.0 * ((double)n.K2 * n.H2 * n.W2 + (double)n.K3 * n.H3 * n.W3) * B;
        }
        return ran != 0;
    }
    void reduce_slabs(const float* slabs, long long slab_stride, int nslab, float* out, long long count) {
        hipLaunchKernelGGL(a0_reduce_slabs_kernel, dim3((unsigned)((count + 31) / 32)), dim3(256), 0, st, slabs, slab_stride, nslab, out, count);
        A0_HIP_THROW(hipGetLastError());
    }
    void reduce_segments(const a0_reduce_seg* segs, int nseg) {
        if (nseg < 1 || nseg > 8) throw std::runtime_error("reduce_segments: 1..8 segments");
        a0_reduce_multi_args A;
        int blocks = 0;
        for (int k = 0; k < 8; ++k) {
            A.first_block[k] = blocks;
            A.vec[k] = 0;
            if (k < nseg) {
                A.seg[k] = segs[k];
                A.vec[k] = ((segs[k].count | segs[k].slab_stride) % 4 == 0) && ((((uintptr_t)segs[k].slabs) | ((uintptr_t)segs[k].out)) % 16 == 0);
                blocks += A.vec[k] ? (int)((segs[k].count / 4 + 31) / 32) : (int)((segs[k].count + 31) / 32);
            } else {
                A.seg[k] = a0_reduce_seg{nullptr, 0, 0, nullptr, 0};
            }
        }
        A.first_block[8] = blocks;
        for (int k = nseg; k < 8; ++k) A.first_block[k] = 0x7fffffff;
        hipLaunchKernelGGL(a0_reduce_segments_kernel, dim3((unsigned)blocks), dim3(256), 0, st, A);
        A0_HIP_THROW(hipGetLastError());
    }
    void reduce_bias_act(const float* slabs, long long slab_stride, int nslab, const float* bias, float* out, int rows, int N, int relu) {
        hipLaunchKernelGGL(a0_reduce_bias_act_kernel, dim3(a0_grid_for((long long)rows * N)), dim3(256), 0, st, slabs, slab_stride, nslab, bias, out, rows, N, relu);
        A0_HIP_THROW(hipGetLastError());
    }
};

struct a0_net {
    a0_net_core core;
    std::vector<void*> owned;
    ~a0_net() { for (void* p : owned) (void)hipFree(p); }
    template <class T> const T* upload(const std::vector<T>& v) {
        void* d = nullptr;
        A0_HIP_THROW(hipMalloc(&d, v.size() * sizeof(T)));
        owned.push_back(d);
        A0_HIP_THROW(hipMemcpy(d, v.data(), v.size() * sizeof(T), hipMemcpyHostToDevice));
        return (const T*)d;
    }
};

extern "C" int a0_net_create(const a0_net_desc* d, a0_net** out) {
    A0_TRY
    if (!d || !out) return a0_fail(A0_EINVAL, "a0_net_create: null argument");
    a0_net* n = new a0_net();
    if (!a0_net_core_init(n->core, d->C, d->H, d->W)) { delete n; return a0_fail(A0_EINVAL, "a0_net_create: observation too small for the 8/4, 4/2, 3/1 conv stack"); }
    a0_net_tables t;
    a0_net_build_tables(n->core, t);
    try {
        n->core.ktab1 = n->upload(t.ktab1); n->core.ktab2 = n->upload(t.ktab2); n->core.ktab3 = n->upload(t.ktab3);
        n->core.ktab_d3 = n->upload(t.ktab_d3); n->core.ktab_d2 = n->upload(t.ktab_d2);
        n->core.wtab_d3 = n->upload(t.wtab_d3);
        for (int i = 0; i < 4; ++i) n->core.wtab_d2[i] = n->upload(t.wtab_d2[i]);
    } catch (...) { delete n; throw; }
    *out = n;
    return A0_OK;
    A0_CATCH
}

extern "C" int a0_net_destroy(a0_net* n) { delete n; return A0_OK; }

extern "C" int a0_net_geometry(const a0_net* n, int* out8) {
    if (!n || !out8) return a0_fail(A0_EINVAL, "a0_net_geometry: null");
    const a0_net_core& c = n->core;
    out8[0] = c.H1; out8[1] = c.W1; out8[2] = c.H2; out8[3] = c.W2; out8[4] = c.H3; out8[5] = c.W3; out8[6] = c.feat; out8[7] = c.K1;
    return A0_OK;
}

extern "C" int a0_net_encoder_fwd(const a0_net* n, const a0_encoder_weights* w, const a0_frames_arg* f, int B,
                                  float* act1, float* act2, float* act3, void* stream) {
    A0_TRY
    if (!n || !w || !f || !f->frames || !act1 || !act2 || !act3 || B < 1) return a0_fail(A0_EINVAL, "a0_net_encoder_fwd: bad argument");
    a0_hip_backend bk{(hipStream_t)stream};
    a0_encoder_fwd_impl(bk, n->core, *w, *f, B, act1, act2, act3);
// ... 410 lines not shown
    a0_mat_src a1{dY, N}, b1{W, K};
    EpiMaskMat::Params e1{dX, X, K};
    a0_mat_src a2{dY, N}, b2{X, ldx};
    EpiWgradSlab::Params e2{grad, 0, K, (long long)N * K};
    a0_mat_src a3{dY2, N2}, b3{X2, ldx2};
    EpiWgradSlab::Params e3{grad2, 0, K2, (long long)N2 * K2};
    A0_HIP_THROW((a0_igemm_x9_trio_launch<OpMatKC, OpMatXC, EpiMaskMat, OpMatXC, OpMatXC, EpiWgradSlab, 4, 2, 1, 1>((hipStream_t)stream, a1, b1, e1, R, K, N, a2, b2, e2, N, K, R,
                                                                                                                  a3, b3, e3, N2, K2, R)));
    return A0_OK;
    A0_CATCH
}

extern "C" long long a0_dense_wgrad_scratch(int R, int N, int K) { return a0_dense_wgrad_scratch_impl(R, N, K); }

extern "C" int a0_dense_wgrad(const float* dY, const float* X, int ldx, float* grad, int R, int N, int K, float* slabs, void* stream) {
    A0_TRY
    if (!dY || !X || !grad || R < 1 || (N & 3) || (K & 3) || (ldx & 3)) return a0_fail(A0_EINVAL, "a0_dense_wgrad: bad shape");
    if (a0_dense_wgrad_scratch_impl(R, N, K) > 0 && !slabs) return a0_fail(A0_EINVAL, "a0_dense_wgrad: needs slab scratch");
    a0_hip_backend bk{(hipStream_t)stream};
    a0_dense_wgrad_impl(bk, dY, X, ldx, grad, R, N, K, slabs);
    return A0_OK;
    A0_CATCH
}

extern "C" int a0_dense_wgrad_multi(int n, const float* const* dY, const float* const* X, const int* ldx, float* const* grad, const int* R, const int* N, const int* K,
                                    float* slabs, const long long* slab_off, a0_pending_reduce* pend, void* stream) {
    A0_TRY
    if (n < 1 || n > 4 || !dY || !X || !ldx || !grad || !R || !N || !K || !slab_off) return a0_fail(A0_EINVAL, "a0_dense_wgrad_multi: 1..4 layers");
    a0_hip_backend bk{(hipStream_t)stream};
    a0_reduce_seg segs[4];
    int nseg = 0;
    for (int i = 0; i < n; ++i) {
        if (!dY[i] || !X[i] || !grad[i] || R[i] < 1 || (N[i] & 3) || (K[i] & 3) || (ldx[i] & 3)) return a0_fail(A0_EINVAL, "a0_dense_wgrad_multi: bad shape");
        if (a0_dense_wgrad_scratch_impl(R[i], N[i], K[i]) > 0 && !slabs) return a0_fail(A0_EINVAL, "a0_dense_wgrad_multi: needs slab scratch");
        a0_reduce_seg seg;
        a0_dense_wgrad_impl(bk, dY[i], X[i], ldx[i], grad[i], R[i], N[i], K[i], slabs ? slabs + slab_off[i] : nullptr, &seg);
        if (seg.nslab > 0) segs[nseg++] = seg;
    }
    if (pend) {
        if (pend->n < 0 || pend->n + nseg > 4) return a0_fail(A0_EINVAL, "a0_dense_wgrad_multi: more than four pending reductions");
        for (int k = 0; k < nseg; ++k) pend->seg[pend->n++] = segs[k];
    } else if (nseg > 0) bk.reduce_segments(segs, nseg);
    return A0_OK;
    A0_CATCH
}

extern "C" int a0_net_encoder_wgrad(const a0_net* n, const a0_encoder_weights* w, const a0_frames_arg* f, int B, const float* act1, const float* act2,
                                    const float* d3, const float* d2, const float* d1, float* g1, float* g2, float* g3, float* slabs, const a0_pending_reduce* pend,
                                    void* stream) {
    A0_TRY
    if (!n || !w || !f || !f->frames || !act1 || !act2 || !d3 || !d2 || !d1 || !g1 || !g2 || !g3 || B < 1) return a0_fail(A0_EINVAL, "a0_net_encoder_wgrad: null argument");
    if (a0_encoder_bwd_scratch_impl(n->core, B) > 0 && !slabs) return a0_fail(A0_EINVAL, "a0_net_encoder_wgrad: needs slab scratch");
    if (pend && (pend->n < 0 || pend->n > 4)) return a0_fail(A0_EINVAL, "a0_net_encoder_wgrad: bad pending reductions");
    a0_hip_backend bk{(hipStream_t)stream};
    a0_encoder_bwd_impl(bk, n->core, *w, *f, B, act1, act2, d3, const_cast<float*>(d2), const_cast<float*>(d1), g1, g2, g3, slabs, false, pend);
    return A0_OK;
    A0_CATCH
}

__global__ void a0_tail_prep_kernel(a0_tail_prep P) {
    if (threadIdx.x == 0 && blockIdx.x == 0) a0_tail_prep_run(P);
}

extern "C" int a0_net_encoder_wgrad_tail(const a0_net* n, const a0_encoder_weights* w, const a0_frames_arg* f, int B, const float* act1, const float* act2,
                                         const float* d3, const float* d2, const float* d1, float* g1, float* g2, float* g3, float* slabs, const a0_pending_reduce* pend,
                                         a0_update_tail_plan* plan, int* state, float* scalars, double lr, double beta1, double beta2, int target_update_freq, void* stream) {
    A0_TRY
    if (!n || !w || !f || !f->frames || !act1 || !act2 || !d3 || !d2 || !d1 || !g1 || !g2 || !g3 || B < 1 || !plan || !state || !scalars)
        return a0_fail(A0_EINVAL, "a0_net_encoder_wgrad_tail: null argument");
    if (a0_encoder_bwd_scratch_impl(n->core, B) > 0 && !slabs) return a0_fail(A0_EINVAL, "a0_net_encoder_wgrad_tail: needs slab scratch");
    if (pend && (pend->n < 0 || pend->n > 4)) return a0_fail(A0_EINVAL, "a0_net_encoder_wgrad_tail: bad pending reductions");
    const a0_tail_prep prep{state, scalars, lr, beta1, beta2, target_update_freq};
    a0_hip_backend bk{(hipStream_t)stream};
    bk.prep = &prep;
    a0_encoder_bwd_impl(bk, n->core, *w, *f, B, act1, act2, d3, const_cast<float*>(d2), const_cast<float*>(d1), g1, g2, g3, slabs, false, pend, plan);
    if (!bk.prep_done) {
        hipLaunchKernelGGL(a0_tail_prep_kernel, dim3(1), dim3(1), 0, (hipStream_t)stream, prep);
        A0_HIP_THROW(hipGetLastError());
    }
    return A0_OK;
    A0_CATCH
}

extern "C" long long a0_net_encoder_bwd_scratch(const a0_net* n, int B) { return n ? a0_encoder_bwd_scratch_impl(n->core, B) : 0; }

extern "C" int a0_net_encoder_bwd(const a0_net* n, const a0_encoder_weights* w, const a0_frames_arg* f, int B,
                                  const float* act1, const float* act2, const float* d3, float* d2, float* d1,
                                  float* g1, float* g2, float* g3, float* slabs, void* stream) {
    A0_TRY
    if (!n || !w || !f || !f->frames || !act1 || !act2 || !d3 || !d2 || !d1 || !g1 || !g2 || !g3 || B < 1) return a0_fail(A0_EINVAL, "a0_net_encoder_bwd: null argument");
    if (a0_encoder_bwd_scratch_impl(n->core, B) > 0 && !slabs) return a0_fail(A0_EINVAL, "a0_net_encoder_bwd: needs slab scratch");
    a0_hip_backend bk{(hipStream_t)stream};
    a0_encoder_bwd_impl(bk, n->core, *w, *f, B, act1, act2, d3, d2, d1, g1, g2, g3, slabs);
    return A0_OK;
    A0_CATCH
}
```

### agent0_amd/deepq/engine.py

```python
from __future__ import annotations

import math
import os
from typing import Dict, List, Optional

import torch

from .layout import Block, NetLayout

MODE_IDENT, MODE_MEAN, MODE_C51, MODE_FQF = 0, 1, 2, 3


def clip_limit(value) -> float:
    return float(value) if value is not None and value > 0 else -1.0


def target_tau_value(value) -> float:
    if value is None or not value > 0:
        return 0.0
    tau = float(value)
    if tau >= 1.0:
        raise ValueError(f"learner.target_tau={tau!r}: must be below 1 (tau >= 1 is the hard copy: leave learner.target_tau off)")
    return tau

# ... 228 lines not shown
            ops.select_action(ws.q, L.A * L.T, L.T, 1, B, L.A, L.T, MODE_C51, atoms, a_star, qsel, qmax)
        elif L.algo == "iqn":
            ops.select_action(ws.q, n_tau * L.A, 1, L.A, B, L.A, n_tau, MODE_MEAN, None, a_star, qsel, qmax)
        else:
            ops.select_action(ws.q, n_tau * L.A, 1, L.A, B, L.A, n_tau, MODE_FQF, ws.tau_all, a_star, qsel, qmax)


class DeviceLearner:

    def __init__(self, ops, L: NetLayout, batch_size: int, *, discount=0.99, n_step=1, double_q=False, lr=5e-4,
                 target_update_freq=500, vmin=-10.0, vmax=10.0, K=32, N=64, N_dash=64, max_grad_norm=-1.0, adam_eps=None,
                 mdqn_tau=0.03, mdqn_lo=-1.0, clip_grad_norm=-1.0, target_tau=0.0):
        self.ops, self.L, self.B = ops, L, batch_size
        self.net = ops.net(L.C, L.H, L.W)
        self.online = DeviceNet(ops, L, self.net)
        self.target = DeviceNet(ops, L, self.net)
        self.noise_joint = None
        if L.noisy and self.online.noise_len % 4 == 0:
            n = self.online.noise_len
            self.noise_joint = ops.zeros(2 * n)
            self.online.adopt_noise_buf(self.noise_joint[:n])
            self.target.adopt_noise_buf(self.noise_joint[n:])
        self.grads = ops.zeros(L.n_params_padded + 4)
        self.adam_m = ops.zeros(L.n_params_padded)
        self.adam_v = ops.zeros(L.n_params_padded)
        self.state = ops.zeros(8, dtype=torch.int32)
        self.scalars = ops.zeros(4)
        self.loss_ring = ops.zeros(1024)
        self.clip_grad_norm = clip_limit(clip_grad_norm)
        self.gnorm_partials = ops.zeros(ops.GRAD_NORM_PARTIALS, dtype=torch.float64) if self.clip_grad_norm > 0 else None
        self.gnorm_ring = ops.zeros(1024) if self.clip_grad_norm > 0 else None
        self.target_tau = target_tau_value(target_tau)
        self.discount, self.n_step, self.double_q = discount, n_step, double_q
        self.gamma_n = float(discount ** n_step)
        self.lr, self.target_update_freq = lr, target_update_freq
        self.adam_eps = (1e-2 / batch_size) if adam_eps is None else adam_eps
        self.vmin, self.vmax = float(vmin), float(vmax)
        self.K, self.N, self.N_dash = K, N, N_dash
        self.max_grad_norm = max_grad_norm
        self.mdqn_tau, self.mdqn_lo = float(mdqn_tau), float(mdqn_lo)
        B = batch_size
        if L.quantile:
            n_on = N if L.algo == "iqn" else L.F
            n_tg = N_dash if L.algo == "iqn" else L.F
            n_sel = K if L.algo == "iqn" else L.F
            self.ws_o = Workspace(ops, L, B, n_on, grads=True)
            self.ws_t = Workspace(ops, L, B, max(n_tg, n_sel))
            self.ws_s = Workspace(ops, L, B, n_sel) if double_q else None
            if L.algo == "fqf":
                self.ws_f = Workspace(ops, L, B, L.F)
                self.rms_sq = ops.zeros(L.blocks["frac"].size)
                self.frac_loss = ops.empty(B)
                self.dfrac_logits = ops.zeros(B * L.Fpad)
                self.clip = ops.zeros(1)
            self.y = ops.empty(B * n_tg)
        else:
            self.ws_o = Workspace(ops, L, B, grads=True)
            self.ws_t = Workspace(ops, L, B)
            self.ws_s = Workspace(ops, L, B) if double_q else None
            if L.algo == "qr":
                self.y = ops.empty(B * L.T)
                self.qr_taus = ((2 * torch.arange(L.T, dtype=torch.float32) + 1) / (2.0 * L.T)).to(ops.device)
            if L.algo == "mdqn":
                self.ws_m = Workspace(ops, L, B)
        if L.algo == "c51":
            self.atoms = torch.linspace(self.vmin, self.vmax, L.T).to(ops.device)
            self.m_proj = ops.empty(B * L.T)
        self.a_star = ops.zeros(B, dtype=torch.int32)
        self.loss = ops.empty(B)
        n_slab = max(ops.encoder_bwd_scratch(self.net, B),
                     ops.dense_wgrad_scratch(self.ws_o.R, L.Npad, 512), ops.dense_wgrad_scratch(self.ws_o.R, 512, L.feat),
                     ops.dense_wgrad_scratch(self.ws_o.R, L.feat, L.num_cosines) if L.quantile else 0,
                     ops.dense_wgrad_scratch(B, L.Fpad, L.feat) if L.algo == "fqf" else 0, 4)
        shapes = [(self.ws_o.R, L.Npad, 512), (self.ws_o.R, 512, L.feat)] + ([(self.ws_o.R, L.feat, L.num_cosines)] if L.quantile else [])
        n_slab = max(n_slab, ops.dense_wgrad_multi_scratch(shapes))
        self._enc_slab_off, self._defer_dense = 0, False
        if hasattr(ops, "pending_reduce") and self.online.fused and self.online.fused_dgrad and os.environ.get("A0_DEFER_DENSE_REDUCE", "1") != "0":
            self._enc_slab_off, self._defer_dense = ops.dense_wgrad_multi_scratch(shapes), True
            n_slab = max(n_slab, self._enc_slab_off + ops.encoder_bwd_scratch(self.net, B))
        self._pend = None
        self.fused_tail = self._defer_dense and hasattr(ops, "update_tail")
        self.fused_tail_reason = "one-launch update tail" if self.fused_tail else "three-launch update tail: the backend has no update_tail or the encoder is not fused"
        self._tail_plan = None
        self.slabs = ops.empty(n_slab)
        self.obs_bytes = L.C * L.H * L.W
        self.grad_hook = None

    def sync_target(self, force=True):
        self.ops.target_sync(self.target.flat, self.online.flat, self.L.n_params_padded, self.state, force)
        self.target.refresh_wt()

    def _hard_freq(self) -> int:
        return 0 if self.target_tau > 0 else self.target_update_freq

    def _blend_target(self, force=False):
        if self.target_tau <= 0:
            return
        L, tg = self.L, self.target
        if tg.fused:
            self.ops.target_blend(tg.flat, self.online.flat, L.n_params_padded, self.target_tau, self.state, self.target_update_freq, force, tg.encoder_weights(), L.C, tg.wt)
        else:
            self.ops.target_blend(tg.flat, self.online.flat, L.n_params_padded, self.target_tau, self.state, self.target_update_freq, force)

    def _grad(self, name: str) -> torch.Tensor:
        L = self.L
        key = name + ".mu" if (L.noisy and name in ("fc1", "head")) else name
        return self.grads[L.blocks[key].all]

    def _backward_dense(self, ws: Workspace, B, have_draw: bool = False, have_dh: bool = False):
        L, ops, on = self.L, self.ops, self.online
        R, T = ws.R, (1 if L.quantile else L.T)
        if not have_draw:
            ops.dueling_bwd(ws.dq, ws.draw, L.Npad, R, L.A, T, L.dueling)
        Wh, _ = on.wb("head")
        Wf, _ = on.wb("fc1")
        wg = [(ws.draw, ws.h, 512, self._grad("head"), R, L.Npad, 512)]
        if not have_dh:
            if hasattr(ops, "dense_dgrad_wgrad_ok2") and ops.dense_dgrad_wgrad_ok2(R, L.Npad, 512):
                ops.dense_dgrad_wgrad(ws.draw, Wh, ws.h, 512, ws.dh, self._grad("head"), R, L.Npad, 512)
                wg = []
            else:
                ops.dense_dgrad(ws.draw, Wh, ws.h, ws.dh, R, L.Npad, 512)
        if not L.quantile:
            if wg and hasattr(ops, "dense_dgrad_wgrad2") and ops.dense_dgrad_wgrad2_ok(R, 512, L.feat, L.Npad, 512):
                ops.dense_dgrad_wgrad2(ws.dh, Wf, ws.act3, L.feat, ws.d3, self._grad("fc1"), R, 512, L.feat, ws.draw, ws.h, 512, self._grad("head"), L.Npad, 512)
                wg = []
            elif hasattr(ops, "dense_dgrad_wgrad") and ops.dense_dgrad_wgrad_ok(R, 512, L.feat):
                ops.dense_dgrad_wgrad(ws.dh, Wf, ws.act3, L.feat, ws.d3, self._grad("fc1"), R, 512, L.feat)
            else:
                wg.append((ws.dh, ws.act3, L.feat, self._grad("fc1"), R, 512, L.feat))
                ops.dense_dgrad(ws.dh, Wf, ws.act3, ws.d3, R, 512, L.feat)
        else:
            n = ws.n_tau
            wg.append((ws.dh, ws.x, L.feat, self._grad("fc1"), R, 512, L.feat))
            if hasattr(ops, "dense_dgrad_hadamard") and ops.dense_dgrad_hadamard_ok(R, 512, L.feat, n):
                ops.dense_dgrad_hadamard(ws.dh, Wf, ws.emb, ws.act3, ws.demb, ws.d3, R, 512, L.feat, n)
            else:
                ops.dense_dgrad(ws.dh, Wf, None, ws.dx, R, 512, L.feat)
                ops.hadamard_bwd(ws.dx, ws.emb, ws.act3, ws.demb, ws.d3, B, n, L.feat)
            wg.append((ws.demb, ws.cosx, L.num_cosines, self._grad("cos"), R, L.feat, L.num_cosines))
        defer = self._defer_dense and self.grad_hook is None
        self._pend = ops.pending_reduce() if defer else None
        if wg:
            ops.dense_wgrad_multi(wg, self.slabs, **({"pend": self._pend} if defer else {}))
        if L.noisy and not defer:
            self._noisy_sigma_grads()

    def _noisy_sigma_grads(self):
        L, on = self.L, self.online
        mods = []
        for prefix, block, r0, r1, in_f in L.noise_modules:
            mu, sg = L.blocks[block + ".mu"], L.blocks[block + ".sigma"]
            nz = on.noise[prefix]
            mods.append((self.grads[mu.all], None, self.grads[sg.all], mu.N, mu.K, r0, r1, nz["noise_in"], nz["noise_out_weight"], nz["noise_out_bias"]))
        self.ops.noisy_multi(True, mods)

    def backward_encoder(self, fuse_tail: bool = False):
        L, ops, on = self.L, self.ops, self.online
        ws, frames, slot, stride, B = self._bw
        g1, g2, g3 = self.grads[L.blocks["conv1"].all], self.grads[L.blocks["conv2"].all], self.grads[L.blocks["conv3"].all]
        self._tail_plan = None
        if on.fused and on.fused_dgrad:
            ops.encoder_dgrad_fused(self.net, on.wt, ws.d3, ws.act1, ws.act2, B, ws.d2, ws.d1)
            pend, self._pend = self._pend, None
            if (fuse_tail and self.fused_tail and pend is not None and self.grad_hook is None and self.clip_grad_norm <= 0 and not (L.noisy and pend.n > 0)):
                self._tail_plan = ops.encoder_wgrad_tail(self.net, on.encoder_weights(), frames, slot, stride, 0, B, ws.act1, ws.act2, ws.d3, ws.d2, ws.d1, g1, g2, g3,
                                                         self.slabs[self._enc_slab_off:], pend, self.state, self.scalars, self.lr, 0.9, 0.999, self._hard_freq())
                if L.noisy:
                    self._noisy_sigma_grads()
            elif pend is not None:
                ops.encoder_wgrad(self.net, on.encoder_weights(), frames, slot, stride, 0, B, ws.act1, ws.act2, ws.d3, ws.d2, ws.d1, g1, g2, g3, self.slabs[self._enc_slab_off:],
                                  pend=pend)
                if L.noisy:
                    self._noisy_sigma_grads()
            else:
                ops.encoder_wgrad(self.net, on.encoder_weights(), frames, slot, stride, 0, B, ws.act1, ws.act2, ws.d3, ws.d2, ws.d1, g1, g2, g3, self.slabs)
        else:
            ops.encoder_bwd(self.net, on.encoder_weights(), frames, slot, stride, 0, B, ws.act1, ws.act2, ws.d3, ws.d2, ws.d1, g1, g2, g3, self.slabs)

    def update(self, frames, slot, sample_stride, act, rew, done, wgt, rand: Optional[List[torch.Tensor]] = None, tstage: Optional[int] = None):
        out = self.forward_dense(frames, slot, sample_stride, act, rew, done, wgt, rand, tstage=tstage)
        self.exchange_begin()
        self.backward_encoder(fuse_tail=True)
        self.exchange_end()
        self.apply()
        return out

    def _bucketed_hook(self) -> bool:
        return self.grad_hook is not None and getattr(self.grad_hook, "bucketed", False)

    def exchange_begin(self):
        h = self.grad_hook
        if self._bucketed_hook():
            h.start_dense(self.grads, self.L.conv_end, self.L.n_params_padded + 1)

    def exchange_end(self):
        h = self.grad_hook
        if h is None:
            return
        if self._bucketed_hook():
            h.finish(self.grads, None, self.L.conv_end)
        else:
            h(self.grads, self.state)

    def forward_backward(self, frames, slot, sample_stride, act, rew, done, wgt, rand: Optional[List[torch.Tensor]] = None):
        out = self.forward_dense(frames, slot, sample_stride, act, rew, done, wgt, rand)
        self.backward_encoder()
        return out

    def apply(self):
        L, ops, on, tg = self.L, self.ops, self.online, self.target
        if L.algo == "fqf":
            blk = L.blocks["frac"]
            ops.rmsprop_step(on.flat[blk.all], self.grads[blk.all], self.rms_sq, blk.size, self.lr / 2e4, 0.95, 1e-5, self.max_grad_norm, self.clip)
        plan, self._tail_plan = self._tail_plan, None
        hard_freq = self._hard_freq()
        if plan is not None:
            ops.update_tail(on.flat, self.grads, self.adam_m, self.adam_v, L.n_adam, self.state, self.scalars, 0.9, 0.999, self.adam_eps, tg.flat, L.n_params_padded, plan,
                            on.encoder_weights(), L.C, on.wt, tg.wt, self.loss, self.B, self.loss_ring)
            self._blend_target()
            return
        tail = self.grads[L.n_params_padded: L.n_params_padded + 1] if self._bucketed_hook() else None
        if self.clip_grad_norm > 0:
            ops.grad_norm_partials(self.grads, L.n_adam, self.gnorm_partials)
            if on.fused:
                ops.adam_step_sync_wt_clip(on.flat, self.grads, self.adam_m, self.adam_v, L.n_adam, self.state, self.scalars, self.lr, 0.9, 0.999, self.adam_eps,
                                           hard_freq, tg.flat, L.n_params_padded, tail, on.encoder_weights(), L.C, on.wt, tg.wt, self.loss, self.B, self.loss_ring,
                                           self.gnorm_partials, self.clip_grad_norm, self.gnorm_ring)
            else:
                ops.adam_step_sync_clip(on.flat, self.grads, self.adam_m, self.adam_v, L.n_adam, self.state, self.scalars, self.lr, 0.9, 0.999, self.adam_eps,
                                        hard_freq, tg.flat, L.n_params_padded, tail, self.gnorm_partials, self.clip_grad_norm, self.gnorm_ring)
            self._blend_target()
            return
        if on.fused:
            ops.adam_step_sync_wt(on.flat, self.grads, self.adam_m, self.adam_v, L.n_adam, self.state, self.scalars, self.lr, 0.9, 0.999, self.adam_eps,
                                  hard_freq, tg.flat, L.n_params_padded, tail, on.encoder_weights(), L.C, on.wt, tg.wt, self.loss, self.B, self.loss_ring)
        else:
            ops.adam_step_sync(on.flat, self.grads, self.adam_m, self.adam_v, L.n_adam, self.state, self.scalars, self.lr, 0.9, 0.999, self.adam_eps,
                               hard_freq, tg.flat, L.n_params_padded, tail)
        self._blend_target()

    def _encode_passes(self, frames, slot, sample_stride, passes):
        L, ops, B = self.L, self.ops, self.B
        multi = len(passes) > 1 and self.online.fused and (L.C, L.H, L.W) == (4, 84, 84) and hasattr(ops, "encoder_fwd_fused_multi")
        if not multi:
            for net, ws, chan_off, keep in passes:
                net.encode(ws, frames, slot, sample_stride, chan_off, B, keep=keep)
            return
# ... 234 lines not shown
```

### agent0_amd/ops.py

```python
from __future__ import annotations

import ctypes as C
from typing import Optional

import torch

from . import _abi
from ._abi import A0Error, EncoderPass, EncoderWeights, FramesArg, LearnerDesc, NetDesc, check


def _stream() -> int:
    return torch._C._cuda_getCurrentRawStream(torch._C._cuda_getDevice())


def _req(t: Optional[torch.Tensor], dtype, min_numel: int, name: str, optional: bool = False):
    if t is None:
        if optional:
            return None
        raise A0Error(f"{name}: tensor required")
    if not t.is_cuda:
        raise A0Error(f"{name}: expected a HIP device tensor (got {t.device}); agent0_amd has no CPU path")
    if t.dtype != dtype:
        raise A0Error(f"{name}: expected {dtype}, got {t.dtype}")
    if not t.is_contiguous():
# ... 141 lines not shown
    def native_learner(self, **kw) -> NativeLearner:
        return NativeLearner(self.lib, **kw)

    def _frames(self, net, frames, slot, sample_stride, chan_off, B):
        hw = net.H * net.W
        need_rows = B if slot is None else 1
        fp = _req(frames, torch.uint8, need_rows * sample_stride if slot is None else chan_off + net.C * hw, "frames")
        if chan_off + net.C * hw > sample_stride:
            raise A0Error("frames: chan_off + C*H*W exceeds sample_stride")
        sp = _req(slot, torch.int32, B, "slot", optional=True)
        return FramesArg(fp, sp, sample_stride, chan_off)

    @staticmethod
    def _enc_w(w):
        return EncoderWeights(*[w[k].data_ptr() for k in ("w1", "b1", "w2", "b2", "w3", "b3")])

    def encoder_fwd(self, net, w, frames, slot, sample_stride, chan_off, B, act1, act2, act3):
        fa = self._frames(net, frames, slot, sample_stride, chan_off, B)
        ew = self._enc_w(w)
        a1 = _req(act1, torch.float32, B * net.H1 * net.W1 * 32, "act1")
        a2 = _req(act2, torch.float32, B * net.H2 * net.W2 * 64, "act2")
        a3 = _req(act3, torch.float32, B * net.feat, "act3")
        check(self.lib.a0_net_encoder_fwd(net.h, C.addressof(ew), C.addressof(fa), B, a1, a2, a3, _stream()), "a0_net_encoder_fwd")

    def fused_supported(self, C_, H, W) -> bool:
        return bool(self.lib.a0_net_encoder_fused_supported(C_, H, W))

    def conv_wt_floats(self, C_) -> int:
        return int(self.lib.a0_net_conv_wt_floats(C_))

    def conv_wt_refresh(self, w, C_, wt):
        ew = self._enc_w(w)
        check(self.lib.a0_net_conv_wt_refresh(C.addressof(ew), C_, _req(wt, torch.float32, self.conv_wt_floats(C_), "wt"), _stream()), "a0_net_conv_wt_refresh")

    def conv_wt_refresh_sync(self, w, C_, wt, wt_target, state):
        ew = self._enc_w(w)
        n = self.conv_wt_floats(C_)
        check(self.lib.a0_net_conv_wt_refresh_sync(C.addressof(ew), C_, _req(wt, torch.float32, n, "wt"), _req(wt_target, torch.float32, n, "wt_target"),
                                                   _req(state, torch.int32, 8, "state"), _stream()), "a0_net_conv_wt_refresh_sync")

    def encoder_fwd_fused(self, net, wt, w, frames, slot, sample_stride, chan_off, B, act1, act2, act3):
        fa = self._frames(net, frames, slot, sample_stride, chan_off, B)
        ew = self._enc_w(w)
        check(self.lib.a0_net_encoder_fwd_fused(net.C, net.H, net.W, _req(wt, torch.float32, self.conv_wt_floats(net.C), "wt"), C.addressof(ew), C.addressof(fa), B,
                                                _req(act1, torch.float32, B * net.H1 * net.W1 * 32, "act1", optional=True),
                                                _req(act2, torch.float32, B * net.H2 * net.W2 * 64, "act2", optional=True),
                                                _req(act3, torch.float32, B * net.feat, "act3"), _stream()), "a0_net_encoder_fwd_fused")

    def encoder_fwd_fused_multi(self, net, passes):
        keep = []
        arr = (EncoderPass * len(passes))()
        for i, (wt, w, frames, slot, sample_stride, chan_off, B, act1, act2, act3) in enumerate(passes):
            fa, ew = self._frames(net, frames, slot, sample_stride, chan_off, B), self._enc_w(w)
            keep += [fa, ew]
            arr[i] = EncoderPass(_req(wt, torch.float32, self.conv_wt_floats(net.C), "wt"), C.addressof(ew), C.addressof(fa), B,
                                 _req(act1, torch.float32, B * net.H1 * net.W1 * 32, "act1", optional=True), _req(act2, torch.float32, B * net.H2 * net.W2 * 64, "act2", optional=True),
                                 _req(act3, torch.float32, B * net.feat, "act3"))
        check(self.lib.a0_net_encoder_fwd_fused_multi(net.C, net.H, net.W, len(passes), C.addressof(arr), _stream()), "a0_net_encoder_fwd_fused_multi")

    def encoder_bwd_scratch(self, net, B) -> int:
        return int(self.lib.a0_net_encoder_bwd_scratch(net.h, B))

    def encoder_bwd(self, net, w, frames, slot, sample_stride, chan_off, B, act1, act2, d3, d2, d1, g1, g2, g3, slabs):
        fa = self._frames(net, frames, slot, sample_stride, chan_off, B)
        ew = self._enc_w(w)
        need = self.encoder_bwd_scratch(net, B)
        check(self.lib.a0_net_encoder_bwd(
            net.h, C.addressof(ew), C.addressof(fa), B,
            _req(act1, torch.float32, B * net.H1 * net.W1 * 32, "act1"), _req(act2, torch.float32, B * net.H2 * net.W2 * 64, "act2"),
            _req(d3, torch.float32, B * net.feat, "d3"), _req(d2, torch.float32, B * net.H2 * net.W2 * 64, "d2"),
            _req(d1, torch.float32, B * net.H1 * net.W1 * 32, "d1"),
            _req(g1, torch.float32, 32 * net.K1 + 32, "g1"), _req(g2, torch.float32, 64 * net.K2 + 64, "g2"), _req(g3, torch.float32, 64 * net.K3 + 64, "g3"),
            _req(slabs, torch.float32, need, "slabs", optional=(need == 0)), _stream()), "a0_net_encoder_bwd")

    def dgrad_fused_supported(self, C_, H, W) -> bool:
        return bool(self.lib.a0_net_encoder_dgrad_fused_supported(C_, H, W))

    def encoder_dgrad_fused(self, net, wt, d3, act1, act2, B, d2, d1):
        check(self.lib.a0_net_encoder_dgrad_fused(net.C, net.H, net.W, _req(wt, torch.float32, self.conv_wt_floats(net.C), "wt"),
                                                  _req(d3, torch.float32, B * net.feat, "d3"), _req(act1, torch.float32, B * net.H1 * net.W1 * 32, "act1"),
                                                  _req(act2, torch.float32, B * net.H2 * net.W2 * 64, "act2"), B,
                                                  _req(d2, torch.float32, B * net.H2 * net.W2 * 64, "d2"), _req(d1, torch.float32, B * net.H1 * net.W1 * 32, "d1"),
                                                  _stream()), "a0_net_encoder_dgrad_fused")

    def pending_reduce(self):
        from ._abi import PendingReduce
        p = PendingReduce()
        p.n = 0
        return p

    def encoder_wgrad(self, net, w, frames, slot, sample_stride, chan_off, B, act1, act2, d3, d2, d1, g1, g2, g3, slabs, pend=None):
        fa = self._frames(net, frames, slot, sample_stride, chan_off, B)
        ew = self._enc_w(w)
        need = self.encoder_bwd_scratch(net, B)
        check(self.lib.a0_net_encoder_wgrad(
            net.h, C.addressof(ew), C.addressof(fa), B,
            _req(act1, torch.float32, B * net.H1 * net.W1 * 32, "act1"), _req(act2, torch.float32, B * net.H2 * net.W2 * 64, "act2"),
            _req(d3, torch.float32, B * net.feat, "d3"), _req(d2, torch.float32, B * net.H2 * net.W2 * 64, "d2"),
            _req(d1, torch.float32, B * net.H1 * net.W1 * 32, "d1"),
            _req(g1, torch.float32, 32 * net.K1 + 32, "g1"), _req(g2, torch.float32, 64 * net.K2 + 64, "g2"), _req(g3, torch.float32, 64 * net.K3 + 64, "g3"),
            _req(slabs, torch.float32, need, "slabs", optional=(need == 0)), None if pend is None else C.addressof(pend), _stream()), "a0_net_encoder_wgrad")

    def encoder_wgrad_tail(self, net, w, frames, slot, sample_stride, chan_off, B, act1, act2, d3, d2, d1, g1, g2, g3, slabs, pend, state, scalars, lr, b1, b2, target_freq):
        from ._abi import UpdateTailPlan
        fa = self._frames(net, frames, slot, sample_stride, chan_off, B)
        ew = self._enc_w(w)
        need = self.encoder_bwd_scratch(net, B)
        plan = UpdateTailPlan()
        plan.n = 0
        check(self.lib.a0_net_encoder_wgrad_tail(
            net.h, C.addressof(ew), C.addressof(fa), B,
            _req(act1, torch.float32, B * net.H1 * net.W1 * 32, "act1"), _req(act2, torch.float32, B * net.H2 * net.W2 * 64, "act2"),
            _req(d3, torch.float32, B * net.feat, "d3"), _req(d2, torch.float32, B * net.H2 * net.W2 * 64, "d2"),
            _req(d1, torch.float32, B * net.H1 * net.W1 * 32, "d1"),
            _req(g1, torch.float32, 32 * net.K1 + 32, "g1"), _req(g2, torch.float32, 64 * net.K2 + 64, "g2"), _req(g3, torch.float32, 64 * net.K3 + 64, "g3"),
            _req(slabs, torch.float32, need, "slabs", optional=(need == 0)), None if pend is None else C.addressof(pend), C.addressof(plan),
            _req(state, torch.int32, 8, "state"), _req(scalars, torch.float32, 2, "scalars"), lr, b1, b2, target_freq, _stream()), "a0_net_encoder_wgrad_tail")
        return plan

    def update_tail(self, params, grads, m, v, n, state, scalars, b1, b2, eps, target, n_total, plan, w, C_, wt, wt_target, loss=None, loss_n=0, loss_ring=None):
        ew = self._enc_w(w)
        nw = self.conv_wt_floats(C_)
        check(self.lib.a0_update_tail(_req(params, torch.float32, n_total, "params"), _req(grads, torch.float32, n_total, "grads"), _req(m, torch.float32, n, "m"),
                                      _req(v, torch.float32, n, "v"), n, _req(state, torch.int32, 8, "state"), _req(scalars, torch.float32, 2, "scalars"),
                                      b1, b2, eps, _req(target, torch.float32, n_total, "target"), n_total, C.addressof(plan), C.addressof(ew), C_,
                                      _req(wt, torch.float32, nw, "wt"), _req(wt_target, torch.float32, nw, "wt_target"),
                                      _req(loss, torch.float32, max(loss_n, 1), "loss", optional=True), int(loss_n), _req(loss_ring, torch.float32, 1, "loss_ring", optional=True),
                                      0 if loss_ring is None else int(loss_ring.numel()), _stream()), "a0_update_tail")

    def dense_fwd_scratch(self, R, N, K) -> int:
        return int(self.lib.a0_dense_fwd_scratch(R, N, K))

    def dense_wgrad_scratch(self, R, N, K) -> int:
        return int(self.lib.a0_dense_wgrad_scratch(R, N, K))

    def dense_fwd(self, X, ldx, W, b, Y, R, N, K, relu, scratch):
        need = self.dense_fwd_scratch(R, N, K)
        check(self.lib.a0_dense_fwd(_req(X, torch.float32, (R - 1) * ldx + K, "X"), ldx, _req(W, torch.float32, N * K, "W"), _req(b, torch.float32, N, "b"),
                                    _req(Y, torch.float32, R * N, "Y"), R, N, K, int(relu),
                                    _req(scratch, torch.float32, need, "scratch", optional=(need == 0)), _stream()), "a0_dense_fwd")

    def dense_fwd_splits(self, R, N, K) -> int:
        return int(self.lib.a0_dense_fwd_splits(R, N, K))

    def dense_fwd_n(self, X, ldx, W, b, Y, R, N, K, relu, splits, scratch):
        need = splits * R * N if splits > 1 else 0
        check(self.lib.a0_dense_fwd_n(_req(X, torch.float32, (R - 1) * ldx + K, "X"), ldx, _req(W, torch.float32, N * K, "W"), _req(b, torch.float32, N, "b"),
                                      _req(Y, torch.float32, R * N, "Y"), R, N, K, int(relu), int(splits),
                                      _req(scratch, torch.float32, need, "scratch", optional=(need == 0)), _stream()), "a0_dense_fwd_n")

    def dense_dgrad_hadamard_ok(self, R, N, K, n) -> bool:
        return bool(self.lib.a0_dense_dgrad_hadamard_ok(R, N, K, n))

    def dense_dgrad_hadamard(self, dY, W, emb, feat, demb, d3, R, N, K, n):
        check(self.lib.a0_dense_dgrad_hadamard(_req(dY, torch.float32, R * N, "dY"), _req(W, torch.float32, N * K, "W"), _req(emb, torch.float32, R * K, "emb"),
                                               _req(feat, torch.float32, (R // n) * K, "feat"), _req(demb, torch.float32, R * K, "demb"), _req(d3, torch.float32, (R // n) * K, "d3"),
                                               R, N, K, n, _stream()), "a0_dense_dgrad_hadamard")

    def weight_planes_words(self, N, K) -> int:
        return int(self.lib.a0_weight_planes_words(N, K))

    def split_planes(self, W, planes, N, K):
        check(self.lib.a0_split_planes(_req(W, torch.float32, N * K, "W"), _req(planes, torch.int32, self.weight_planes_words(N, K), "planes"), N, K, _stream()), "a0_split_planes")

    def dense_fwd_wplanes_ok(self, R, N, K) -> bool:
        return bool(self.lib.a0_dense_fwd_wplanes_ok(R, N, K))

    def dense_fwd_wplanes(self, X, ldx, planes, b, Y, R, N, K, relu):
        check(self.lib.a0_dense_fwd_wplanes(_req(X, torch.float32, (R - 1) * ldx + K, "X"), ldx, _req(planes, torch.int32, self.weight_planes_words(N, K), "planes"),
                                            _req(b, torch.float32, N, "b"), _req(Y, torch.float32, R * N, "Y"), R, N, K, int(relu), _stream()), "a0_dense_fwd_wplanes")

    def dense_fwd_mul(self, X, ldx, W, b, M, group, Y, R, N, K, relu):
        check(self.lib.a0_dense_fwd_mul(_req(X, torch.float32, (R - 1) * ldx + K, "X"), ldx, _req(W, torch.float32, N * K, "W"), _req(b, torch.float32, N, "b"),
                                        _req(M, torch.float32, ((R - 1) // group + 1) * N, "M"), group, _req(Y, torch.float32, R * N, "Y"), R, N, K, int(relu), _stream()),
              "a0_dense_fwd_mul")

    def dense_fwd_mul_keep_ok(self, R, N, K, ldx) -> bool:
        return bool(self.lib.a0_dense_fwd_mul_keep_ok(R, N, K, ldx))

    def dense_fwd_mul_keep(self, X, ldx, W, b, M, group, E, Y, R, N, K, relu):
        check(self.lib.a0_dense_fwd_mul_keep(_req(X, torch.float32, (R - 1) * ldx + K, "X"), ldx, _req(W, torch.float32, N * K, "W"), _req(b, torch.float32, N, "b"),
                                             _req(M, torch.float32, ((R - 1) // group + 1) * N, "M"), group, _req(E, torch.float32, R * N, "E"),
                                             _req(Y, torch.float32, R * N, "Y"), R, N, K, int(relu), _stream()), "a0_dense_fwd_mul_keep")

    def dense_dgrad(self, dY, W, mask, dX, R, N, K):
        check(self.lib.a0_dense_dgrad(_req(dY, torch.float32, R * N, "dY"), _req(W, torch.float32, N * K, "W"),
                                      _req(mask, torch.float32, R * K, "mask", optional=True), _req(dX, torch.float32, R * K, "dX"), R, N, K, _stream()), "a0_dense_dgrad")

    def dense_wgrad(self, dY, X, ldx, grad, R, N, K, slabs):
        need = self.dense_wgrad_scratch(R, N, K)
        check(self.lib.a0_dense_wgrad(_req(dY, torch.float32, R * N, "dY"), _req(X, torch.float32, (R - 1) * ldx + K, "X"), ldx,
                                      _req(grad, torch.float32, N * K + N, "grad"), R, N, K,
                                      _req(slabs, torch.float32, need, "slabs", optional=(need == 0)), _stream()), "a0_dense_wgrad")

    def dueling_fwd(self, raw, ld, q, R, A, T, dueling):
        check(self.lib.a0_dueling_fwd(_req(raw, torch.float32, R * ld, "raw"), ld, _req(q, torch.float32, R * A * T, "q"), R, A, T, int(dueling), _stream()), "a0_dueling_fwd")

    def dueling_bwd(self, dq, draw, ld, R, A, T, dueling):
        check(self.lib.a0_dueling_bwd(_req(dq, torch.float32, R * A * T, "dq"), _req(draw, torch.float32, R * ld, "draw"), ld, R, A, T, int(dueling), _stream()), "a0_dueling_bwd")

# ... 691 lines not shown
```

### include/agent0_hip.h

```cpp
#ifndef AGENT0_HIP_H
#define AGENT0_HIP_H

#include <stdint.h>

#ifdef __cplusplus
extern "C" {
#endif

#define A0_ABI_VERSION 1

#define A0_CTRL_ENV_STEP 0
#define A0_CTRL_ACTOR_STEPS 1
#define A0_CTRL_RNG_ACTION 2
#define A0_CTRL_RNG_UNIFORM 3
#define A0_CTRL_REPLAY_SLOT 4
#define A0_CTRL_RNG_TAUS 5
#define A0_CTRL_RNG_NOISE 6
#define A0_CTRL_WORDS 8

const char* a0_last_error(void);
int a0_abi_version(void);
const char* a0_build_info(void);
int a0_device_info(int* cu_count, long long* hbm_bytes, char* arch_name64);

typedef struct a0_net_desc {
    int C, H, W;
} a0_net_desc;

typedef struct a0_net a0_net;

typedef struct a0_frames_arg {
    const uint8_t* frames;
    const int* slot;
    long long sample_stride;
    int chan_off;
} a0_frames_arg;

typedef struct a0_reduce_seg { const float* slabs; long long slab_stride; int nslab; float* out; long long count; } a0_reduce_seg;
typedef struct a0_pending_reduce { a0_reduce_seg seg[4]; int n; } a0_pending_reduce;

typedef struct a0_encoder_weights {
    const float *w1, *b1, *w2, *b2, *w3, *b3;
} a0_encoder_weights;

typedef struct a0_encoder_pass {
    const float* wt; const a0_encoder_weights* w; const a0_frames_arg* f; int B;
    float *act1, *act2, *act3;
} a0_encoder_pass;

int a0_net_create(const a0_net_desc* desc, a0_net** out);
int a0_net_destroy(a0_net* net);
int a0_net_geometry(const a0_net* net, int* out8);

int a0_net_encoder_fwd(const a0_net* net, const a0_encoder_weights* w, const a0_frames_arg* frames, int B,
                       float* act1, float* act2, float* act3, void* stream);

int a0_net_encoder_fused_supported(int C, int H, int W);
long long a0_net_conv_wt_floats(int C);
int a0_net_conv_wt_refresh(const a0_encoder_weights* w, int C, float* wt, void* stream);
int a0_net_conv_wt_refresh_sync(const a0_encoder_weights* w, int C, float* wt, float* wt_target, const int* state, void* stream);
int a0_net_encoder_fwd_fused(int C, int H, int W, const float* wt, const a0_encoder_weights* w, const a0_frames_arg* frames, int B,
                             float* act1, float* act2, float* act3, void* stream);
int a0_net_encoder_fwd_fused_multi(int C, int H, int W, int n, const a0_encoder_pass* pass, void* stream);

int a0_net_encoder_dgrad_fused_supported(int C, int H, int W);
int a0_net_encoder_dgrad_fused(int C, int H, int W, const float* wt, const float* d3, const float* act1, const float* act2, int B, float* d2,
                               float* d1, void* stream);

long long a0_net_encoder_bwd_scratch(const a0_net* net, int B);
int a0_net_encoder_bwd(const a0_net* net, const a0_encoder_weights* w, const a0_frames_arg* frames, int B,
                       const float* act1, const float* act2, const float* d3, float* d2, float* d1,
                       float* g1, float* g2, float* g3, float* slabs, void* stream);

int a0_net_encoder_wgrad(const a0_net* net, const a0_encoder_weights* w, const a0_frames_arg* frames, int B, const float* act1, const float* act2,
                         const float* d3, const float* d2, const float* d1, float* g1, float* g2, float* g3, float* slabs, const a0_pending_reduce* pend,
                         void* stream);

typedef struct a0_update_tail_plan { a0_reduce_seg seg[8]; int n; } a0_update_tail_plan;
int a0_net_encoder_wgrad_tail(const a0_net* net, const a0_encoder_weights* w, const a0_frames_arg* frames, int B, const float* act1, const float* act2,
                              const float* d3, const float* d2, const float* d1, float* g1, float* g2, float* g3, float* slabs, const a0_pending_reduce* pend,
                              a0_update_tail_plan* plan, int* state, float* scalars2, double lr, double beta1, double beta2, int target_update_freq, void* stream);

long long a0_dense_fwd_scratch(int R, int N, int K);
int a0_dense_fwd(const float* X, int ldx, const float* W, const float* b, float* Y, int R, int N, int K, int relu,
                 float* scratch, void* stream);
int a0_dense_fwd_splits(int R, int N, int K);
int a0_dense_fwd_n(const float* X, int ldx, const float* W, const float* b, float* Y, int R, int N, int K, int relu, int splits, float* scratch, void* stream);
int a0_dense_dgrad(const float* dY, const float* W, const float* act_mask, float* dX, int R, int N, int K, void* stream);
int a0_dense_dgrad_wgrad_ok(int R, int N, int K);
int a0_dense_dgrad_wgrad_ok2(int R, int N, int K);
int a0_dense_dgrad_wgrad(const float* dY, const float* W, const float* X, int ldx, float* dX, float* grad_w_b, int R, int N, int K, void* stream);
int a0_dense_dgrad_wgrad2_ok(int R, int N, int K, int N2, int K2);
int a0_dense_dgrad_wgrad2(const float* dY, const float* W, const float* X, int ldx, float* dX, float* grad, int R, int N, int K,
                          const float* dY2, const float* X2, int ldx2, float* grad2, int N2, int K2, void* stream);
long long a0_dense_wgrad_scratch(int R, int N, int K);
int a0_dense_wgrad(const float* dY, const float* X, int ldx, float* grad_w_b, int R, int N, int K, float* slabs, void* stream);
int a0_dense_wgrad_multi(int n, const float* const* dY, const float* const* X, const int* ldx, float* const* grad_w_b, const int* R, const int* N, const int* K,
                         float* slabs, const long long* slab_off, a0_pending_reduce* pend, void* stream);

int a0_dense_fwd_mul(const float* X, int ldx, const float* W, const float* b, const float* M, int group, float* Y, int R, int N, int K, int relu, void* stream);

int a0_dense_fwd_mul_keep_ok(int R, int N, int K, int ldx);
int a0_dense_fwd_mul_keep(const float* X, int ldx, const float* W, const float* b, const float* M, int group, float* E, float* Y, int R, int N, int K, int relu, void* stream);

int a0_dense_fwd_partial_slabs(int R, int N, int K);
int a0_dense_fwd_partial(const float* X, int ldx, const float* W, int R, int N, int K, float* slabs, void* stream);
int a0_dense_fwd_partial_n(const float* X, int ldx, const float* W, int R, int N, int K, int splits, float* slabs, void* stream);
int a0_dense_fwd_partial_multi_ok(int n, int R, int N, int K);
int a0_dense_fwd_partial_multi_slabs(int n, int R, int N, int K);
int a0_dense_fwd_partial_multi(int n, const float* const* X, int ldx, const float* const* W, int R, int N, int K, float* const* slabs, const long long* slab_stride,
                               void* stream);
int a0_reduce_bias_act_multi(int n, const float* const* slabs, const long long* slab_stride, const int* nslab, const float* const* bias, float* const* out,
                             const int* rows, int N, int relu, void* stream);

int a0_probe_begin(int tag, int max_launches);
int a0_probe_end(double* host_out3);

int a0_trace_enabled(void);
int a0_trace_rank(int rank);
int a0_trace_push(const char* name);
int a0_trace_pop(void);

long long a0_weight_planes_words(int N, int K);
int a0_split_planes(const float* W, unsigned int* planes, int N, int K, void* stream);
int a0_dense_fwd_wplanes_ok(int R, int N, int K);
int a0_dense_fwd_wplanes(const float* X, int ldx, const unsigned int* Wplanes, const float* b, float* Y, int R, int N, int K, int relu, void* stream);

int a0_gemm_mode(int mode);

int a0_x9_products(int n);

int a0_dueling_fwd(const float* raw, int ld, float* q, int R, int A, int T, int dueling, void* stream);
int a0_dueling_bwd(const float* dq, float* draw, int ld, int R, int A, int T, int dueling, void* stream);

int a0_select_action(const float* x, long long sb, long long sa, long long st, int B, int A, int T, int mode,
                     const float* aux, int* a_star, float* qsel, float* qmax, void* stream);
int a0_actor_dist_tail(const float* slabs, long long slab_stride, int nslab, const float* bias, int ld, int A, int T, int dueling, int mode,
                       const float* atoms, int E, unsigned long long seed, unsigned int stream_a, unsigned int stream_u, unsigned long long off_a,
                       unsigned long long off_u, float eps, const long long* ctrl, const float* eps_ptr, int* action, float* qmax, void* stream);
int a0_actor_quantile_tail(const float* slabs, long long slab_stride, int nslab, const float* bias, int ld, int A, int T, int dueling, int mode,
                           const float* taus, int E, unsigned long long seed, unsigned int stream_a, unsigned int stream_u, unsigned long long off_a,
                           unsigned long long off_u, float eps, const long long* ctrl, const float* eps_ptr, int* action, float* qmax, void* stream);
int a0_actor_dist_tail_env_step(const float* slabs, long long slab_stride, int nslab, const float* bias, int ld, int A, int T, int dueling, int mode,
                                const float* atoms, int E, unsigned long long seed, unsigned int stream_a, unsigned int stream_u, unsigned long long off_a,
                                unsigned long long off_u, float eps, const long long* ctrl, const float* eps_ptr, int* action, float* qmax,
                                unsigned long long env_seed, unsigned int rank, unsigned int g, const uint8_t* obs_in, uint8_t* obs_out, float* ep_ret,
                                float* final_mask, float* final_ret, int n, long long steps, double gamma, int* ring_act, float* ring_rew, float* ring_done,
                                const uint8_t* obs0, uint8_t* frames, long long cap, long long start_slot, int* r_act, float* r_rew, float* r_done, int task, void* stream);

int a0_actor_quantile_tail_env_step(const float* slabs, long long slab_stride, int nslab, const float* bias, int ld, int A, int T, int dueling, int mode,
                                    const float* taus, int E, unsigned long long seed, unsigned int stream_a, unsigned int stream_u, unsigned long long off_a,
                                    unsigned long long off_u, float eps, const long long* ctrl, const float* eps_ptr, int* action, float* qmax,
                                    unsigned long long env_seed, unsigned int rank, unsigned int g, const uint8_t* obs_in, uint8_t* obs_out, float* ep_ret,
                                    float* final_mask, float* final_ret, int n, long long steps, double gamma, int* ring_act, float* ring_rew, float* ring_done,
                                    const uint8_t* obs0, uint8_t* frames, long long cap, long long start_slot, int* r_act, float* r_rew, float* r_done, int task, void* stream);

int a0_loss_dqn(const float* q, const float* q_next, int A, const int* act, const int* a_star, const float* rew,
                const float* done, const float* wgt, float gamma_n, int B, float* loss, float* dq, int* nan_flag, void* stream);
int a0_dqn_head_loss(const float* h_on, const float* h_tg, const float* h_sel, const float* W_on, const float* b_on, const float* W_tg,
                     const float* b_tg, int A, int dueling, int ld, const int* act, const float* rew, const float* done, const float* wgt,
                     float gamma_n, int B, float* loss, float* q_on_out, float* q_tg_out, float* draw, int* nan_flag, void* stream);
int a0_dqn_head_loss_slabs(const float* slabs_on, const float* slabs_tg, const float* slabs_sel, long long slab_stride, int nslab, const float* b1_on,
                           const float* b1_tg, float* h_on_out, const float* W_on, const float* b_on, const float* W_tg, const float* b_tg, int A,
                           int dueling, int ld, const int* act, const float* rew, const float* done, const float* wgt, float gamma_n, int B, float* loss,
// ... 313 lines not shown
```

Measured before the change: 2.340 million.

## Emit pre-split bf16 gradient planes from dgrad and consume them in conv2/3 wgrad

The fused dgrad kernel now also writes the hi/mid/lo bf16 split of the conv2 and conv3 output gradients to global plane buffers. The conv2/3 wgrad kernel can then load these planes directly instead of re-reading fp32 gradients and re-splitting them for each part. Only the bias-owning part keeps the fp32 path so it can still compute bias sums. The change targets redundant split arithmetic and fp32 load traffic in wgrad, at the cost of extra global writes in dgrad, extra buffer memory, and more kernel template variants.

```diff
diff --git a/agent0_amd/csrc/a0_internal.h b/agent0_amd/csrc/a0_internal.h
--- a/agent0_amd/csrc/a0_internal.h
+++ b/agent0_amd/csrc/a0_internal.h
@@ -59,8 +59,8 @@
             hipLaunchKernelGGL(kern, grid, block, lds, st, __VA_ARGS__);                                                           \
     } while (0)
 struct a0_net_core;
-int a0_conv23_wgrad_fused_launch(const a0_net_core& n, int B, const float* act1, const float* act2, const float* d2, const float* d3, float* slab2, float* slab3,
-                                 hipStream_t st);
+int a0_conv23_wgrad_fused_launch(const a0_net_core& n, int B, const float* act1, const float* act2, const float* d2, const float* d3, const void* d2p, const void* d3p,
+                                 float* slab2, float* slab3, hipStream_t st);
 #endif
 #define A0_TAG_ENCODER_FUSED 12
 #define A0_TAG_ENCODER_DGRAD_FUSED 13
diff --git a/agent0_amd/csrc/conv23_wgrad.hip b/agent0_amd/csrc/conv23_wgrad.hip
--- a/agent0_amd/csrc/conv23_wgrad.hip
+++ b/agent0_amd/csrc/conv23_wgrad.hip
@@ -14,6 +14,7 @@
 
 struct a0_c23w_args {
     const float *act1, *act2, *d2, *d3;
+    const unsigned char *d2p, *d3p;
     float *slab2, *slab3;
     int B, G2, G3;
 };
@@ -23,12 +24,14 @@
     static constexpr int NPOS = 81, STEPS = 5, DROWS = 96, APIX = 100, CIN = 32, K = 512;
     static constexpr int ACT_PLANE = APIX * A0Q_ROW, D_PLANE = 2 * DROWS * A0Q_ROW;
     static constexpr int ACT_F4 = 100 * 8, D_F4 = 81 * 16;
+    static constexpr int DG_PLANE = 2 * NPOS * A0Q_ROW;
     A0_D static int base_row(int p) { return 10 * (p / 9) + (p % 9); }
 };
 template <> struct a0q_geom<3> {
     static constexpr int NPOS = 49, STEPS = 3, DROWS = 64, APIX = 81, CIN = 64, K = 576;
     static constexpr int ACT_PLANE = 2 * APIX * A0Q_ROW, D_PLANE = 2 * DROWS * A0Q_ROW;
     static constexpr int ACT_F4 = 81 * 16, D_F4 = 49 * 16;
+    static constexpr int DG_PLANE = 2 * NPOS * A0Q_ROW;
     A0_D static int base_row(int p) { return 9 * (p / 7) + (p % 7); }
 };
 constexpr int A0Q_LDS_BYTES = 3 * (a0q_geom<2>::ACT_PLANE + a0q_geom<2>::D_PLANE);
@@ -57,11 +60,18 @@
     return a0q_u32x4{a.x, a.y, b.x, b.y};
 }
 
-template <int NPR, int LAYER, int NT>
+template <int LAYER>
+A0_D int a0q_boff(int lane, int s, int h) {
+    const int p = 16 * s + 8 * (lane >> 5) + ((lane & 15) >> 2) + 4 * h;
+    return a0q_geom<LAYER>::base_row(p) * A0Q_ROW + 2 * (16 * ((lane >> 4) & 1) + 4 * (lane & 3));
+}
+
+template <int NPR, int LAYER, int NT, bool RB>
 A0_D void a0q_mma_steps(const unsigned char* act, const unsigned char* dpl, int aoff, const int (&boff)[a0q_geom<LAYER>::STEPS][2],
                         int a_blk, const int (&b_blk)[2], a0_acc16 (&acc)[2]) {
     typedef a0q_geom<LAYER> G;
-    const int lane = threadIdx.x & 63;
+    int lane = threadIdx.x & 63;
+    if constexpr (RB) asm volatile("" : "+v"(lane));
     constexpr int TA[9] = {2, 2, 1, 2, 1, 0, 1, 0, 0};
     constexpr int TB[9] = {2, 1, 2, 0, 1, 2, 0, 1, 0};
 #pragma unroll
@@ -71,7 +81,8 @@
         for (int t = 0; t < 3; ++t) {
             a[t] = a0q_frag(dpl + t * G::D_PLANE + a_blk + s * 16 * A0Q_ROW, aoff, aoff + 4 * A0Q_ROW);
 #pragma unroll
-            for (int j = 0; j < NT; ++j) b[j][t] = a0q_frag(act + t * G::ACT_PLANE + b_blk[j], boff[s][0], boff[s][1]);
+            for (int j = 0; j < NT; ++j)
+                b[j][t] = a0q_frag(act + t * G::ACT_PLANE + b_blk[j], RB ? a0q_boff<LAYER>(lane, s, 0) : boff[s][0], RB ? a0q_boff<LAYER>(lane, s, 1) : boff[s][1]);
         }
 #pragma unroll
         for (int q = 9 - NPR; q < 9; ++q)
@@ -96,7 +107,7 @@
     }
 }
 
-template <int NPR, int LAYER>
+template <int NPR, int LAYER, bool PL>
 A0_D void a0q_body(const a0_c23w_args& P, int part, int g, int ngroups, unsigned char* smem) {
     typedef a0q_geom<LAYER> G;
     const int tid = threadIdx.x, lane = tid & 63;
@@ -125,14 +136,12 @@
     }
     const int colb = 2 * (16 * ((lane >> 4) & 1) + 4 * (lane & 3));
     const int aoff = (8 * (lane >> 5) + ((lane & 15) >> 2)) * A0Q_ROW + colb;
+    constexpr bool RB = PL && LAYER == 3;
     int boff[G::STEPS][2];
 #pragma unroll
     for (int s = 0; s < G::STEPS; ++s)
 #pragma unroll
-        for (int h = 0; h < 2; ++h) {
-            const int p = 16 * s + 8 * (lane >> 5) + ((lane & 15) >> 2) + 4 * h;
-            boff[s][h] = G::base_row(p) * A0Q_ROW + colb;
-        }
+        for (int h = 0; h < 2; ++h) boff[s][h] = RB ? 0 : a0q_boff<LAYER>(lane, s, h);
 
     a0_acc16 acc[2];
 #pragma unroll
@@ -142,7 +151,10 @@
     float bsum[4] = {0.f, 0.f, 0.f, 0.f};
 
     constexpr int RA = (G::ACT_F4 + A0Q_THREADS - 1) / A0Q_THREADS, RD = (G::D_F4 + A0Q_THREADS - 1) / A0Q_THREADS;
-    a0_f4 ra[RA], rd[RD];
+    a0_f4 ra[RA], rd[PL ? 1 : RD];
+    a0q_u32x2 rp[PL ? RD : 1][3];
+    const bool has_bias = !PL && part == 0;
+    const int doff = (((tid & 15) >> 3) * G::NPOS + (tid >> 4)) * A0Q_ROW + (tid & 7) * 8;
     auto load_raw = [&](int b) {
         const float* sa = LAYER == 2 ? P.act1 + (long long)b * (400 * 32) : P.act2 + (long long)b * (81 * 64);
 #pragma unroll
@@ -154,9 +166,19 @@
                 ra[j] = *(const a0_f4*)(sa + ((2 * r + (part >> 1)) * 20 + 2 * c + (part & 1)) * 32 + (i & 7) * 4);
             } else ra[j] = *(const a0_f4*)(sa + i * 4);
         }
-        const a0_f4* sd = (const a0_f4*)((LAYER == 2 ? P.d2 : P.d3) + (long long)b * (G::NPOS * 64));
-#pragma unroll
-        for (int j = 0; j < RD; ++j) { const int i = tid + j * A0Q_THREADS; rd[j] = sd[i < G::D_F4 ? i : G::D_F4 - 1]; }
+        if constexpr (PL) {
+            const unsigned char* sp = (LAYER == 2 ? P.d2p : P.d3p) + (long long)b * (3 * G::DG_PLANE);
+#pragma unroll
+            for (int j = 0; j < RD; ++j) {
+                const int off = tid + j * A0Q_THREADS < G::D_F4 ? doff + j * (A0Q_THREADS / 16) * A0Q_ROW : doff;
+#pragma unroll
+                for (int t = 0; t < 3; ++t) rp[j][t] = *(const a0q_u32x2*)(sp + t * G::DG_PLANE + off);
+            }
+        } else {
+            const a0_f4* sd = (const a0_f4*)((LAYER == 2 ? P.d2 : P.d3) + (long long)b * (G::NPOS * 64));
+#pragma unroll
+            for (int j = 0; j < RD; ++j) { const int i = tid + j * A0Q_THREADS; rd[j] = sd[i < G::D_F4 ? i : G::D_F4 - 1]; }
+        }
     };
     int b = g;
     if (b < P.B) load_raw(b);
@@ -180,17 +202,21 @@
             const int i = tid + j * A0Q_THREADS;
             if (i < G::D_F4) {
                 const int c4 = (i & 15) * 4, row = (c4 >> 5) * G::DROWS + (i >> 4), cb = (c4 & 31) * 2;
-                bsum[0] += rd[j].x; bsum[1] += rd[j].y; bsum[2] += rd[j].z; bsum[3] += rd[j].w;
                 a0q_u32x2 hi, mid, lo;
-                a0q_split4(rd[j], hi, mid, lo);
+                if constexpr (PL) {
+                    hi = rp[j][0]; mid = rp[j][1]; lo = rp[j][2];
+                } else {
+                    bsum[0] += rd[j].x; bsum[1] += rd[j].y; bsum[2] += rd[j].z; bsum[3] += rd[j].w;
+                    a0q_split4(rd[j], hi, mid, lo);
+                }
                 unsigned char* d = dpl + row * A0Q_ROW + cb;
                 *(a0q_u32x2*)d = hi; *(a0q_u32x2*)(d + G::D_PLANE) = mid; *(a0q_u32x2*)(d + 2 * G::D_PLANE) = lo;
             }
         }
         __syncthreads();
         if (b + ngroups < P.B) load_raw(b + ngroups);
-        if (nt == 2) a0q_mma_steps<NPR, LAYER, 2>(act, dpl, aoff, boff, a_blk, b_blk, acc);
-        else a0q_mma_steps<NPR, LAYER, 1>(act, dpl, aoff, boff, a_blk, b_blk, acc);
+        if (nt == 2) a0q_mma_steps<NPR, LAYER, 2, RB>(act, dpl, aoff, boff, a_blk, b_blk, acc);
+        else a0q_mma_steps<NPR, LAYER, 1, RB>(act, dpl, aoff, boff, a_blk, b_blk, acc);
         __syncthreads();
     }
 
@@ -205,7 +231,6 @@
             }
         }
     }
-    const bool has_bias = part == 0;
     if (has_bias) {
         float* red = (float*)smem;
 #pragma unroll
@@ -220,27 +245,36 @@
     }
 }
 
-template <int NPR>
+template <int NPR, bool PL>
 __global__ __launch_bounds__(A0Q_THREADS, 4) void a0_conv23_wgrad_fused_kernel(a0_c23w_args P) {
     extern __shared__ __attribute__((aligned(16))) unsigned char a0q_smem[];
     const int xcd = blockIdx.x & 7, k = blockIdx.x >> 3, g = xcd + 8 * (k / 7), part = k % 7;
     if (g >= P.G2) return;
-    if (part < 4) a0q_body<NPR, 2>(P, part, g, P.G2, a0q_smem);
-    else a0q_body<NPR, 3>(P, part - 4, g, P.G3, a0q_smem);
-}
-
-int a0_conv23_wgrad_fused_launch(const a0_net_core& n, int B, const float* act1, const float* act2, const float* d2, const float* d3, float* slab2, float* slab3,
-                                 hipStream_t st) {
+    if constexpr (PL) {
+        if (part == 0) a0q_body<NPR, 2, false>(P, 0, g, P.G2, a0q_smem);
+        else if (part < 4) a0q_body<NPR, 2, true>(P, part, g, P.G2, a0q_smem);
+        else if (part == 4) a0q_body<NPR, 3, false>(P, 0, g, P.G3, a0q_smem);
+        else a0q_body<NPR, 3, true>(P, part - 4, g, P.G3, a0q_smem);
+    } else {
+        if (part < 4) a0q_body<NPR, 2, false>(P, part, g, P.G2, a0q_smem);
+        else a0q_body<NPR, 3, false>(P, part - 4, g, P.G3, a0q_smem);
+    }
+}
+
+int a0_conv23_wgrad_fused_launch(const a0_net_core& n, int B, const float* act1, const float* act2, const float* d2, const float* d3, const void* d2p, const void* d3p,
+                                 float* slab2, float* slab3, hipStream_t st) {
     int G2 = 0, G3 = 0;
     if (!a0_c23w_plan(n, B, &G2, &G3) || !slab2 || !slab3) return 0;
     a0_c23w_args P;
-    P.act1 = act1; P.act2 = act2; P.d2 = d2; P.d3 = d3; P.slab2 = slab2; P.slab3 = slab3; P.B = B; P.G2 = G2; P.G3 = G3;
+    P.act1 = act1; P.act2 = act2; P.d2 = d2; P.d3 = d3; P.d2p = (const unsigned char*)d2p; P.d3p = (const unsigned char*)d3p; P.slab2 = slab2; P.slab3 = slab3; P.B = B; P.G2 = G2; P.G3 = G3;
     const int six = a0_x9_products_now() == 6;
-    auto kern = six ? a0_conv23_wgrad_fused_kernel<6> : a0_conv23_wgrad_fused_kernel<9>;
-    static bool configured[2] = {false, false};
-    if (!configured[six]) {
+    const int pl = d2p != nullptr && d3p != nullptr;
+    auto kern = pl ? (six ? a0_conv23_wgrad_fused_kernel<6, true> : a0_conv23_wgrad_fused_kernel<9, true>)
+                   : (six ? a0_conv23_wgrad_fused_kernel<6, false> : a0_conv23_wgrad_fused_kernel<9, false>);
+    static bool configured[2][2] = {{false, false}, {false, false}};
+    if (!configured[pl][six]) {
         A0_HIP_THROW(hipFuncSetAttribute((const void*)kern, hipFuncAttributeMaxDynamicSharedMemorySize, A0Q_LDS_BYTES));
-        configured[six] = true;
+        configured[pl][six] = true;
     }
     if (G2 != G3) return 0;
     hipLaunchKernelGGL(kern, dim3(8 * 7 * ((G2 + 7) / 8)), dim3(A0Q_THREADS), A0Q_LDS_BYTES, st, P);
diff --git a/agent0_amd/csrc/encoder_fused.hip b/agent0_amd/csrc/encoder_fused.hip
--- a/agent0_amd/csrc/encoder_fused.hip
+++ b/agent0_amd/csrc/encoder_fused.hip
@@ -985,11 +985,13 @@
 struct a0_dgrad_args {
     const float *d3, *act1, *act2;
     float *d2, *d1;
+    uint16_t *d2p, *d3p;
     const float *wd3, *wd2;
     int B;
 };
 constexpr int A0_RPDA = 11 * A0_P2X + 96, A0_RPDB = 11 * A0_P2X + 48;
 constexpr int A0_DTERMA = 11 * A0_RPDA, A0_DTERMB = 11 * A0_RPDB;
+constexpr int A0_D2P_TERM = 2 * 81 * 32, A0_D3P_TERM = 2 * 49 * 32;
 struct AFD3X {
     static constexpr int term = A0_DTERMA;
     const uint16_t* planes;
@@ -1006,7 +1008,7 @@
     static constexpr bool PER_ELEM = true;
     static constexpr bool ROW4 = false;
     static constexpr bool TR = true;
-    const float* mask; float* dst; uint16_t* planes;
+    const float* mask; float* dst; uint16_t* planes; uint16_t* gpl;
     A0_D a0_f4 pre_elem4(int m, int n0) const { return *(const a0_f4*)(mask + (unsigned)(m * 64 + n0)); }
     A0_D void emit_n4(int m, int n0, const a0_acc4& acc, const float* pre) const {
         float v[4];
@@ -1018,6 +1020,10 @@
         const int oh = m / 9, ow = m - oh * 9;
         uint16_t* d = planes + (oh + 1) * A0_RPDB + (ow + 1) * A0_P2X + n0;
         *(uint2*)d = hi; *(uint2*)(d + A0_DTERMB) = mid; *(uint2*)(d + 2 * A0_DTERMB) = lo;
+        if (gpl) {
+            uint16_t* g = gpl + ((n0 >> 5) * 81 + m) * 32 + (n0 & 31);
+            *(uint2*)g = hi; *(uint2*)(g + A0_D2P_TERM) = mid; *(uint2*)(g + 2 * A0_D2P_TERM) = lo;
+        }
     }
 };
 static_assert((A0_RPDB % 4) == 0 && (A0_DTERMB % 4) == 0 && (A0_P2X % 4) == 0, "8-byte aligned plane writes");
@@ -1060,11 +1066,15 @@
             a0_split4(x, hi, mid, lo);
             uint16_t* d = plA + (h + 2) * A0_RPDA + (w + 2) * A0_P2X + c4;
             *(uint2*)(d) = hi; *(uint2*)(d + A0_DTERMA) = mid; *(uint2*)(d + 2 * A0_DTERMA) = lo;
+            if (P.d3p) {
+                uint16_t* g = P.d3p + (long long)b * (3 * A0_D3P_TERM) + ((c4 >> 5) * 49 + pos) * 32 + (c4 & 31);
+                *(uint2*)(g) = hi; *(uint2*)(g + A0_D3P_TERM) = mid; *(uint2*)(g + 2 * A0_D3P_TERM) = lo;
+            }
         }
         __syncthreads();
         const AFD3X f3{plA};
         const AFD2X f2{plB};
-        const EpiBwd3X e3{P.act2 + (long long)b * 81 * 64, P.d2 + (long long)b * 81 * 64, plB};
+        const EpiBwd3X e3{P.act2 + (long long)b * 81 * 64, P.d2 + (long long)b * 81 * 64, plB, P.d2p ? P.d2p + (long long)b * (3 * A0_D2P_TERM) : nullptr};
         const EpiBwdPair e2a{P.act1 + (long long)b * 400 * 32, P.d1 + (long long)b * 400 * 32, 0};
         const EpiBwdPair e2b{P.act1 + (long long)b * 400 * 32, P.d1 + (long long)b * 400 * 32, 2};
         a0_conv_stage_x9k<ORD, 64, 4, 6, 3, 1>(f3, 81, ring3, e3, xch0, xch1, [&] { ringq[0].init_at(wq, 4, 768); ringq[0].prologue(); });
@@ -1253,13 +1263,13 @@
 
 extern "C" int a0_net_encoder_dgrad_fused_supported(int C, int H, int W) { return (C >= 1 && H == 84 && W == 84) ? 1 : 0; }
 
-extern "C" int a0_net_encoder_dgrad_fused(int C, int H, int W, const float* wt, const float* d3, const float* act1, const float* act2, int B, float* d2,
-                                          float* d1, void* stream) {
+static int a0_encoder_dgrad_fused_run(int C, int H, int W, const float* wt, const float* d3, const float* act1, const float* act2, int B, float* d2, float* d1,
+                                      uint16_t* d2p, uint16_t* d3p, void* stream) {
     A0_TRY
     if (!wt || !d3 || !act1 || !act2 || !d2 || !d1 || B < 1) return a0_fail(A0_EINVAL, "a0_net_encoder_dgrad_fused: bad argument");
     if (!a0_net_encoder_dgrad_fused_supported(C, H, W)) return a0_fail(A0_EINVAL, "a0_net_encoder_dgrad_fused: 84x84 observations only");
     a0_dgrad_args P;
-    P.d3 = d3; P.act1 = act1; P.act2 = act2; P.d2 = d2; P.d1 = d1; P.B = B;
+    P.d3 = d3; P.act1 = act1; P.act2 = act2; P.d2 = d2; P.d1 = d1; P.d2p = d2p; P.d3p = d3p; P.B = B;
     P.wd3 = wt + a0_wt_layout{C}.dgrad3x(); P.wd2 = wt + a0_wt_layout{C}.dgrad2x();
     const size_t lds = (size_t)3 * (A0_DTERMA + A0_DTERMB) * 2 + (4 * 4 + 4 * 3) * 1024;
     static bool configured[2] = {false, false};
@@ -1275,3 +1285,14 @@
     return A0_OK;
     A0_CATCH
 }
+
+extern "C" int a0_net_encoder_dgrad_fused(int C, int H, int W, const float* wt, const float* d3, const float* act1, const float* act2, int B, float* d2,
+                                          float* d1, void* stream) {
+    return a0_encoder_dgrad_fused_run(C, H, W, wt, d3, act1, act2, B, d2, d1, nullptr, nullptr, stream);
+}
+
+extern "C" int a0_net_encoder_dgrad_fused_planes(int C, int H, int W, const float* wt, const float* d3, const float* act1, const float* act2, int B, float* d2,
+                                                 float* d1, void* d2_planes, void* d3_planes, void* stream) {
+    if (!d2_planes || !d3_planes) return a0_fail(A0_EINVAL, "a0_net_encoder_dgrad_fused_planes: bad argument");
+    return a0_encoder_dgrad_fused_run(C, H, W, wt, d3, act1, act2, B, d2, d1, (uint16_t*)d2_planes, (uint16_t*)d3_planes, stream);
+}
diff --git a/agent0_amd/csrc/learner.hip b/agent0_amd/csrc/learner.hip
--- a/agent0_amd/csrc/learner.hip
+++ b/agent0_amd/csrc/learner.hip
@@ -111,6 +111,7 @@
         const long long Rg = fqf ? (long long)B * d->fqf_F : (iqn ? (long long)B * d->iqn_N : (long long)B);
         L->draw = L->alloc<float>(Rg * L->Npad); L->dh = L->alloc<float>(Rg * 512); L->d3 = L->alloc<float>((long long)B * L->feat);
         L->d2 = L->alloc<float>((long long)B * L->H2 * L->W2 * 64); L->d1 = L->alloc<float>((long long)B * L->H1 * L->W1 * 32); L->loss = L->alloc<float>(B);
+        L->d2p = L->alloc<uint16_t>((long long)B * L->H2 * L->W2 * 64 * 3); L->d3p = L->alloc<uint16_t>((long long)B * L->feat * 3);
         const long long s_head = ceil_to(a0_dense_wgrad_scratch((int)Rg, L->Npad, 512), 4), s_fc1 = ceil_to(a0_dense_wgrad_scratch((int)Rg, 512, L->feat), 4);
         const long long s_cos = iqn ? ceil_to(a0_dense_wgrad_scratch((int)Rg, L->feat, 64), 4) : 0;
         L->slab_off[0] = 0; L->slab_off[1] = s_head;
@@ -626,16 +627,12 @@
             A0_CHECK(a0_dp_allreduce(L->dp_comm, L->grads + conv_end, L->n_pad + 1 - conv_end, L->dp_side));
         }
     }
-    A0_CHECK(a0_net_encoder_dgrad_fused(L->C, L->H, L->W, L->wt_on, L->d3, L->act1, L->act2, B, L->d2, L->d1, stream));
+    A0_CHECK(a0_net_encoder_dgrad_fused_planes(L->C, L->H, L->W, L->wt_on, L->d3, L->act1, L->act2, B, L->d2, L->d1, L->d2p, L->d3p, stream));
     a0_update_tail_plan tail;
     const bool fuse_tail = !dp && L->clip_max_norm <= 0.f && !(L->d.noisy && pend.n > 0);
-    if (fuse_tail)
-        A0_CHECK(a0_net_encoder_wgrad_tail(L->net, &w_on, &f_obs, B, L->act1, L->act2, L->d3, L->d2, L->d1, L->grads + L->conv1.off, L->grads + L->conv2.off,
-                                           L->grads + L->conv3.off, L->slabs + L->enc_slab_off, &pend, &tail, L->state, L->scalars, L->d.lr, 0.9, 0.999,
-                                           hard_freq, stream));
-    else
-    A0_CHECK(a0_net_encoder_wgrad(L->net, &w_on, &f_obs, B, L->act1, L->act2, L->d3, L->d2, L->d1, L->grads + L->conv1.off, L->grads + L->conv2.off, L->grads + L->conv3.off,
-                                  L->slabs + L->enc_slab_off, &pend, stream));
+    A0_CHECK(a0_net_encoder_wgrad_planes(L->net, &w_on, &f_obs, B, L->act1, L->act2, L->d3, L->d2, L->d1, L->d2p, L->d3p, L->grads + L->conv1.off, L->grads + L->conv2.off,
+                                         L->grads + L->conv3.off, L->slabs + L->enc_slab_off, &pend, fuse_tail ? &tail : nullptr, L->state, L->scalars, L->d.lr, 0.9, 0.999,
+                                         hard_freq, stream));
     if (dp) {
         if (dp_inline) {
             A0_CHECK(a0_dp_allreduce(L->dp_comm, L->grads, conv_end, stream));
diff --git a/agent0_amd/csrc/learner_state.h b/agent0_amd/csrc/learner_state.h
--- a/agent0_amd/csrc/learner_state.h
+++ b/agent0_amd/csrc/learner_state.h
@@ -70,6 +70,7 @@
     float *act1 = nullptr, *act2 = nullptr, *act3_o = nullptr, *act3_t = nullptr, *act3_s = nullptr;
     float *fc1_slabs[3] = {nullptr, nullptr, nullptr};
     float *h = nullptr, *q_o = nullptr, *q_t = nullptr, *draw = nullptr, *dh = nullptr, *d3 = nullptr, *d2 = nullptr, *d1 = nullptr, *loss = nullptr, *slabs = nullptr;
+    uint16_t *d2p = nullptr, *d3p = nullptr;
     std::vector<void*> owned;
     long long dp_comm = 0;
     hipStream_t dp_side = nullptr;
diff --git a/agent0_amd/csrc/net.hip b/agent0_amd/csrc/net.hip
--- a/agent0_amd/csrc/net.hip
+++ b/agent0_amd/csrc/net.hip
@@ -194,6 +194,7 @@
     int tag = 0;
     const a0_tail_prep* prep = nullptr;
     bool prep_done = false;
+    const void *d2p = nullptr, *d3p = nullptr;
     template <class OA, class OB, class EP, int WM, int WN, int MT, int NT>
     void igemm(const typename OA::Params& pa, const typename OB::Params& pb, const typename EP::Params& pe, int X, int Y, int K, int splits) {
         hipEvent_t e0 = nullptr, e1 = nullptr;
@@ -253,7 +254,7 @@
     bool conv23_wgrad_fused(const a0_net_core& n, int B, const float* act1, const float* act2, const float* d2, const float* d3, float* slab2, float* slab3) {
         const bool probe = g_probe.tag != 0 && g_probe.tag == A0_TAG_CONV2_WGRAD && g_probe.used + 2 <= g_probe.ev.size();
         if (probe) A0_HIP_THROW(hipEventRecord(g_probe.ev[g_probe.used], st));
-        const int ran = a0_conv23_wgrad_fused_launch(n, B, act1, act2, d2, d3, slab2, slab3, st);
+        const int ran = a0_conv23_wgrad_fused_launch(n, B, act1, act2, d2, d3, d2p, d3p, slab2, slab3, st);
         if (probe && ran) {
             A0_HIP_THROW(hipEventRecord(g_probe.ev[g_probe.used + 1], st));
             g_probe.used += 2;
@@ -830,6 +831,28 @@
     A0_CATCH
 }
 
+extern "C" int a0_net_encoder_wgrad_planes(const a0_net* n, const a0_encoder_weights* w, const a0_frames_arg* f, int B, const float* act1, const float* act2,
+                                           const float* d3, const float* d2, const float* d1, const void* d2_planes, const void* d3_planes, float* g1, float* g2, float* g3,
+                                           float* slabs, const a0_pending_reduce* pend, a0_update_tail_plan* plan, int* state, float* scalars, double lr, double beta1,
+                                           double beta2, int target_update_freq, void* stream) {
+    A0_TRY
+    if (!n || !w || !f || !f->frames || !act1 || !act2 || !d3 || !d2 || !d1 || !d2_planes || !d3_planes || !g1 || !g2 || !g3 || B < 1 || (plan && (!state || !scalars)))
+        return a0_fail(A0_EINVAL, "a0_net_encoder_wgrad_planes: null argument");
+    if (a0_encoder_bwd_scratch_impl(n->core, B) > 0 && !slabs) return a0_fail(A0_EINVAL, "a0_net_encoder_wgrad_planes: needs slab scratch");
+    if (pend && (pend->n < 0 || pend->n > 4)) return a0_fail(A0_EINVAL, "a0_net_encoder_wgrad_planes: bad pending reductions");
+    const a0_tail_prep prep{state, scalars, lr, beta1, beta2, target_update_freq};
+    a0_hip_backend bk{(hipStream_t)stream};
+    bk.d2p = d2_planes; bk.d3p = d3_planes;
+    if (plan) bk.prep = &prep;
+    a0_encoder_bwd_impl(bk, n->core, *w, *f, B, act1, act2, d3, const_cast<float*>(d2), const_cast<float*>(d1), g1, g2, g3, slabs, false, pend, plan);
+    if (plan && !bk.prep_done) {
+        hipLaunchKernelGGL(a0_tail_prep_kernel, dim3(1), dim3(1), 0, (hipStream_t)stream, prep);
+        A0_HIP_THROW(hipGetLastError());
+    }
+    return A0_OK;
+    A0_CATCH
+}
+
 extern "C" long long a0_net_encoder_bwd_scratch(const a0_net* n, int B) { return n ? a0_encoder_bwd_scratch_impl(n->core, B) : 0; }
 
 extern "C" int a0_net_encoder_bwd(const a0_net* n, const a0_encoder_weights* w, const a0_frames_arg* f, int B,
diff --git a/agent0_amd/deepq/engine.py b/agent0_amd/deepq/engine.py
--- a/agent0_amd/deepq/engine.py
+++ b/agent0_amd/deepq/engine.py
@@ -334,6 +334,10 @@
         self.fused_tail = self._defer_dense and hasattr(ops, "update_tail")
         self.fused_tail_reason = "one-launch update tail" if self.fused_tail else "three-launch update tail: the backend has no update_tail or the encoder is not fused"
         self._tail_plan = None
+        self.wgrad_planes = (self.online.fused and self.online.fused_dgrad and hasattr(ops, "encoder_dgrad_fused_planes") and hasattr(ops, "encoder_wgrad_planes"))
+        if self.wgrad_planes:
+            self.d2_planes = ops.empty(B * L.H2 * L.W2 * 64 * 3, dtype=torch.bfloat16)
+            self.d3_planes = ops.empty(B * L.feat * 3, dtype=torch.bfloat16)
         self.slabs = ops.empty(n_slab)
         self.obs_bytes = L.C * L.H * L.W
         self.grad_hook = None
@@ -413,9 +417,18 @@
         g1, g2, g3 = self.grads[L.blocks["conv1"].all], self.grads[L.blocks["conv2"].all], self.grads[L.blocks["conv3"].all]
         self._tail_plan = None
         if on.fused and on.fused_dgrad:
+            pend, self._pend = self._pend, None
+            tail = fuse_tail and self.fused_tail and pend is not None and self.grad_hook is None and self.clip_grad_norm <= 0 and not (L.noisy and pend.n > 0)
+            if self.wgrad_planes:
+                ops.encoder_dgrad_fused_planes(self.net, on.wt, ws.d3, ws.act1, ws.act2, B, ws.d2, ws.d1, self.d2_planes, self.d3_planes)
+                self._tail_plan = ops.encoder_wgrad_planes(self.net, on.encoder_weights(), frames, slot, stride, 0, B, ws.act1, ws.act2, ws.d3, ws.d2, ws.d1,
+                                                           self.d2_planes, self.d3_planes, g1, g2, g3, self.slabs[self._enc_slab_off:] if pend is not None else self.slabs,
+                                                           pend, tail, self.state, self.scalars, self.lr, 0.9, 0.999, self._hard_freq())
+                if L.noisy and pend is not None:
+                    self._noisy_sigma_grads()
+                return
             ops.encoder_dgrad_fused(self.net, on.wt, ws.d3, ws.act1, ws.act2, B, ws.d2, ws.d1)
-            pend, self._pend = self._pend, None
-            if (fuse_tail and self.fused_tail and pend is not None and self.grad_hook is None and self.clip_grad_norm <= 0 and not (L.noisy and pend.n > 0)):
+            if tail:
                 self._tail_plan = ops.encoder_wgrad_tail(self.net, on.encoder_weights(), frames, slot, stride, 0, B, ws.act1, ws.act2, ws.d3, ws.d2, ws.d1, g1, g2, g3,
                                                          self.slabs[self._enc_slab_off:], pend, self.state, self.scalars, self.lr, 0.9, 0.999, self._hard_freq())
                 if L.noisy:
diff --git a/agent0_amd/ops.py b/agent0_amd/ops.py
--- a/agent0_amd/ops.py
+++ b/agent0_amd/ops.py
@@ -247,6 +247,14 @@
                                                   _req(act2, torch.float32, B * net.H2 * net.W2 * 64, "act2"), B,
                                                   _req(d2, torch.float32, B * net.H2 * net.W2 * 64, "d2"), _req(d1, torch.float32, B * net.H1 * net.W1 * 32, "d1"),
                                                   _stream()), "a0_net_encoder_dgrad_fused")
+
+    def encoder_dgrad_fused_planes(self, net, wt, d3, act1, act2, B, d2, d1, d2_planes, d3_planes):
+        check(self.lib.a0_net_encoder_dgrad_fused_planes(net.C, net.H, net.W, _req(wt, torch.float32, self.conv_wt_floats(net.C), "wt"),
+                                                         _req(d3, torch.float32, B * net.feat, "d3"), _req(act1, torch.float32, B * net.H1 * net.W1 * 32, "act1"),
+                                                         _req(act2, torch.float32, B * net.H2 * net.W2 * 64, "act2"), B,
+                                                         _req(d2, torch.float32, B * net.H2 * net.W2 * 64, "d2"), _req(d1, torch.float32, B * net.H1 * net.W1 * 32, "d1"),
+                                                         _req(d2_planes, torch.bfloat16, B * net.H2 * net.W2 * 64 * 3, "d2_planes"),
+                                                         _req(d3_planes, torch.bfloat16, B * net.feat * 3, "d3_planes"), _stream()), "a0_net_encoder_dgrad_fused_planes")
 
     def pending_reduce(self):
         from ._abi import PendingReduce
@@ -281,6 +289,28 @@
             _req(g1, torch.float32, 32 * net.K1 + 32, "g1"), _req(g2, torch.float32, 64 * net.K2 + 64, "g2"), _req(g3, torch.float32, 64 * net.K3 + 64, "g3"),
             _req(slabs, torch.float32, need, "slabs", optional=(need == 0)), None if pend is None else C.addressof(pend), C.addressof(plan),
             _req(state, torch.int32, 8, "state"), _req(scalars, torch.float32, 2, "scalars"), lr, b1, b2, target_freq, _stream()), "a0_net_encoder_wgrad_tail")
+        return plan
+
+    def encoder_wgrad_planes(self, net, w, frames, slot, sample_stride, chan_off, B, act1, act2, d3, d2, d1, d2_planes, d3_planes, g1, g2, g3, slabs, pend=None, tail=False,
+                             state=None, scalars=None, lr=0.0, b1=0.0, b2=0.0, target_freq=0):
+        from ._abi import UpdateTailPlan
+        fa = self._frames(net, frames, slot, sample_stride, chan_off, B)
+        ew = self._enc_w(w)
+        need = self.encoder_bwd_scratch(net, B)
+        plan = None
+        if tail:
+            plan = UpdateTailPlan()
+            plan.n = 0
+        check(self.lib.a0_net_encoder_wgrad_planes(
+            net.h, C.addressof(ew), C.addressof(fa), B,
+            _req(act1, torch.float32, B * net.H1 * net.W1 * 32, "act1"), _req(act2, torch.float32, B * net.H2 * net.W2 * 64, "act2"),
+            _req(d3, torch.float32, B * net.feat, "d3"), _req(d2, torch.float32, B * net.H2 * net.W2 * 64, "d2"),
+            _req(d1, torch.float32, B * net.H1 * net.W1 * 32, "d1"),
+            _req(d2_planes, torch.bfloat16, B * net.H2 * net.W2 * 64 * 3, "d2_planes"), _req(d3_planes, torch.bfloat16, B * net.feat * 3, "d3_planes"),
+            _req(g1, torch.float32, 32 * net.K1 + 32, "g1"), _req(g2, torch.float32, 64 * net.K2 + 64, "g2"), _req(g3, torch.float32, 64 * net.K3 + 64, "g3"),
+            _req(slabs, torch.float32, need, "slabs", optional=(need == 0)), None if pend is None else C.addressof(pend), None if plan is None else C.addressof(plan),
+            _req(state, torch.int32, 8, "state", optional=not tail), _req(scalars, torch.float32, 2, "scalars", optional=not tail), lr, b1, b2, target_freq, _stream()),
+            "a0_net_encoder_wgrad_planes")
         return plan
 
     def update_tail(self, params, grads, m, v, n, state, scalars, b1, b2, eps, target, n_total, plan, w, C_, wt, wt_target, loss=None, loss_n=0, loss_ring=None):
diff --git a/include/agent0_hip.h b/include/agent0_hip.h
--- a/include/agent0_hip.h
+++ b/include/agent0_hip.h
@@ -66,6 +66,8 @@
 int a0_net_encoder_dgrad_fused_supported(int C, int H, int W);
 int a0_net_encoder_dgrad_fused(int C, int H, int W, const float* wt, const float* d3, const float* act1, const float* act2, int B, float* d2,
                                float* d1, void* stream);
+int a0_net_encoder_dgrad_fused_planes(int C, int H, int W, const float* wt, const float* d3, const float* act1, const float* act2, int B, float* d2,
+                                      float* d1, void* d2_planes, void* d3_planes, void* stream);
 
 long long a0_net_encoder_bwd_scratch(const a0_net* net, int B);
 int a0_net_encoder_bwd(const a0_net* net, const a0_encoder_weights* w, const a0_frames_arg* frames, int B,
@@ -80,6 +82,11 @@
 int a0_net_encoder_wgrad_tail(const a0_net* net, const a0_encoder_weights* w, const a0_frames_arg* frames, int B, const float* act1, const float* act2,
                               const float* d3, const float* d2, const float* d1, float* g1, float* g2, float* g3, float* slabs, const a0_pending_reduce* pend,
                               a0_update_tail_plan* plan, int* state, float* scalars2, double lr, double beta1, double beta2, int target_update_freq, void* stream);
+
+int a0_net_encoder_wgrad_planes(const a0_net* net, const a0_encoder_weights* w, const a0_frames_arg* frames, int B, const float* act1, const float* act2,
+                                const float* d3, const float* d2, const float* d1, const void* d2_planes, const void* d3_planes, float* g1, float* g2, float* g3,
+                                float* slabs, const a0_pending_reduce* pend, a0_update_tail_plan* plan, int* state, float* scalars2, double lr, double beta1, double beta2,
+                                int target_update_freq, void* stream);
 
 long long a0_dense_fwd_scratch(int R, int N, int K);
 int a0_dense_fwd(const float* X, int ldx, const float* W, const float* b, float* Y, int R, int N, int K, int relu,
```

Result: no change. 2.321 million (-0.8%).
